# dvalcarce/filmyou-core

Hardware: AMD Instinct MI355X
Metric: top-N recs/sec (RM2), ml25m shape (higher is better)
Workload: dtype f32 (scores and logs fp32 / v_log_f32, folded in fp64; co-rating sums 64-bit fixed point in LDS (fp64 fallback); G stored as 24-bit e7m17 floats scaled per cluster above 4096 items; ratings fp16 in the row kernel when exactly representable)

## Files before the change

### filmyou-core_amd/csrc/fy_cooc.hpp

```cpp
#pragma once
#include <hip/hip_fp16.h>

#include <type_traits>

#include "fy_common.hpp"

namespace fy {

struct CoocArgs {
    const int32_t* __restrict__ rank_pair;
    const int32_t* __restrict__ pair_start;
    const int32_t* __restrict__ seg_ptr;
    const int2* __restrict__ seg;
    const float* __restrict__ seg_w;
    const int32_t* __restrict__ csr_idx;
    const float* __restrict__ csr_w;
    int32_t pbase;
    int32_t slot_base;
    int32_t Ic;
    int32_t CH;
    int32_t nch;
    int32_t row0;
    int32_t nrows;
    int32_t q0;
    int32_t nq;
    const int32_t* __restrict__ local_start;
    int32_t row_stride;
    const uint32_t* __restrict__ csr_pk;
    const int2* __restrict__ item_seg;
    uint32_t pk_bytes;
    const int32_t* __restrict__ item_id;
    int32_t half;
    double fx_scale;
    int32_t tail_row0, tail_chunks;
    int32_t item_grab;
    int32_t acc_quarter;
    int32_t acc32;
    int32_t half_rows, head_chunks;
};
__device__ __forceinline__ bool cooc_row_is_cut(const CoocArgs& A, int row) { return A.half && (A.half_rows == 0 || row < A.half_rows); }
__device__ __forceinline__ int cooc_acc_index(int c, int quarter) { return quarter ? (c & 3) * quarter + (c >> 2) : c; }

#ifndef FY_COOC_NB
#define FY_COOC_NB 8
#endif
extern __shared__ __attribute__((aligned(16))) double fy_cooc_acc[];

struct SegBatch {
    int2 d;
    float w;
};
static_assert(FY_COOC_NB == 8, "the segment groups of cooc_seg_slot are 8 segments long");
__device__ __forceinline__ int cooc_seg_slot(int s_begin, int batch, int wave, int nwaves, int lane) {
    return s_begin + ((((batch << 3) + (lane >> 3)) * nwaves + wave) << 3) + (lane & 7);
}
__device__ __forceinline__ SegBatch cooc_first_batch(const CoocArgs& A, int s_begin, int s_end) {
    const int lane = threadIdx.x & 63;
    const int wave = __builtin_amdgcn_readfirstlane(threadIdx.x >> 6);
    SegBatch B{make_int2(0, 0), 0.0f};
    const int s = cooc_seg_slot(s_begin, 0, wave, blockDim.x >> 6, lane);
    if (s < s_end) { B.d = A.seg[s]; B.w = A.seg_w[s]; }
    return B;
}

template <bool PK, class ACC>
__device__ __forceinline__ void cooc_accumulate_segments(const CoocArgs& A, ACC* __restrict__ acc, int s_begin, int s_end, int c0, SegBatch first,
                                                         int rmask = -1 ) {
    const int lane = threadIdx.x & 63;
    const int wave = __builtin_amdgcn_readfirstlane(threadIdx.x >> 6);
    const int nwaves = blockDim.x >> 6;
    const int32_t* __restrict__ csr_idx = A.csr_idx;
    const float* __restrict__ csr_w = A.csr_w;
    const uint32_t* __restrict__ csr_pk = A.csr_pk;
    constexpr int NB = FY_COOC_NB;
    struct Group {
        int L[NB];
        float W[NB];
        int idx[NB];
        float x[NB];
    };
    auto issue = [&](Group& G, const int2& d, float w, int g) __attribute__((always_inline)) {
#pragma unroll
        for (int q = 0; q < NB; q++) {
            const int F = __builtin_amdgcn_readlane(d.x, g + q);
            G.L[q] = __builtin_amdgcn_readlane(d.y, g + q);
            G.W[q] = __uint_as_float(__builtin_amdgcn_readlane(__float_as_uint(w), g + q));
            const int at = F + (lane < G.L[q] ? lane : 0);
            G.x[q] = 0.0f;
            if constexpr (PK) G.idx[q] = (int)csr_pk[at];
            else {
                G.idx[q] = csr_idx[at] - c0;
                G.x[q] = csr_w[at];
            }
        }
    };
    auto commit = [&](Group& G) __attribute__((always_inline)) {
        if constexpr (PK) {
#pragma unroll
            for (int q = 0; q < NB; q++) {
                const uint32_t pk = (uint32_t)G.idx[q];
                G.x[q] = __half2float(__ushort_as_half((unsigned short)(pk >> 16)));
                G.idx[q] = (int)(pk & 0xFFFFu);
            }
        }
#pragma unroll
        for (int q = 0; q < NB; q++)
            if (lane < G.L[q] && G.idx[q] > rmask) atomicAdd(&acc[cooc_acc_index(G.idx[q], A.acc_quarter)], (ACC)G.W[q] * (ACC)G.x[q]);
    };
    int batch = 0;
    if (cooc_seg_slot(s_begin, 0, wave, nwaves, 0) >= s_end) return;
    int2 d = first.d;
    float w = first.w;
    while (true) {
        const int nloc = __popcll(__ballot(cooc_seg_slot(s_begin, batch, wave, nwaves, lane) < s_end));
        const int s_next = cooc_seg_slot(s_begin, batch + 1, wave, nwaves, lane);
        int2 dn = make_int2(0, 0);
        float wn = 0.0f;
        if (s_next < s_end) { dn = A.seg[s_next]; wn = A.seg_w[s_next]; }
        Group GA, GB;
        issue(GA, d, w, 0);
#pragma unroll 1
        for (int g = 0; g < 64; g += 2 * NB) {
            issue(GB, d, w, g + NB);
            commit(GA);
            if (g + 2 * NB < 64) issue(GA, d, w, g + 2 * NB);
            commit(GB);
            if (g + 2 * NB >= nloc) break;
        }
        d = dn;
        w = wn;
        batch++;
        if (cooc_seg_slot(s_begin, batch, wave, nwaves, 0) >= s_end) break;
    }
}

struct PkGroup {
    int L[FY_COOC_NB];
    float W[FY_COOC_NB];
    uint32_t pk[FY_COOC_NB];
};
__device__ __forceinline__ void cooc_pk_issue(const __amdgpu_buffer_rsrc_t rsrc, int lane4, PkGroup& G, const int2& d, float w, int g) {
#pragma unroll
    for (int q = 0; q < FY_COOC_NB; q++) {
        const int F = __builtin_amdgcn_readlane(d.x, g + q);
        G.L[q] = __builtin_amdgcn_readlane(d.y, g + q);
        G.W[q] = __uint_as_float(__builtin_amdgcn_readlane(__float_as_uint(w), g + q));
        G.pk[q] = (uint32_t)__builtin_amdgcn_raw_buffer_load_b32(rsrc, lane4, F * 4, 0);
    }
}
__device__ __forceinline__ __amdgpu_buffer_rsrc_t cooc_pk_rsrc(const CoocArgs& A) {
    return __builtin_amdgcn_make_buffer_rsrc(const_cast<uint32_t*>(A.csr_pk), 0, (int)A.pk_bytes, 0x00020000);
}
template <class ACC>
__device__ __forceinline__ void cooc_accumulate_pk(const CoocArgs& A, ACC* __restrict__ acc, int s_begin, int s_end, SegBatch first,
                                                   int rmask = -1 ) {
    const int lane = threadIdx.x & 63;
    const int wave = __builtin_amdgcn_readfirstlane(threadIdx.x >> 6);
    const int nwaves = blockDim.x >> 6;
    const __amdgpu_buffer_rsrc_t rsrc = cooc_pk_rsrc(A);
    const int lane4 = lane * 4;
    constexpr int NB = FY_COOC_NB;
    using Group = PkGroup;
    auto issue = [&](Group& G, const int2& d, float w, int g) __attribute__((always_inline)) { cooc_pk_issue(rsrc, lane4, G, d, w, g); };
    const double fx = A.fx_scale;
    const uint32_t ix_mask = A.acc_quarter ? 3u : 0u, ix_shift = A.acc_quarter ? 2u : 0u, ix_quarter = (uint32_t)A.acc_quarter;
    auto commit = [&](Group& G) __attribute__((always_inline)) {
#pragma unroll
        for (int q = 0; q < NB; q++) {
            const float x = __half2float(__ushort_as_half((unsigned short)(G.pk[q] >> 16)));
            if constexpr (std::is_same<ACC, uint32_t>::value) {
                const uint32_t v = (uint32_t)(G.W[q] * x * (float)fx);
                if (lane < G.L[q] && (int)(G.pk[q] & 0xFFFFu) > rmask) atomicAdd(&acc[cooc_acc_index((int)(G.pk[q] & 0xFFFFu), A.acc_quarter)], v);
            } else if constexpr (std::is_same<ACC, unsigned long long>::value) {
                const double d = fma((double)(G.W[q] * x), fx, 4503599627370496.0);
                unsigned long long v = (unsigned long long)__double_as_longlong(d) & 0xFFFFFFFFFFFFFull;
                const uint32_t c = G.pk[q] & 0xFFFFu;
                uint32_t at = __umul24(c & ix_mask, ix_quarter) + (c >> ix_shift);
                asm volatile("" : "+v"(at), "+v"(v));
                if (lane < G.L[q] && (int)c > rmask) atomicAdd(&acc[at], v);
            } else {
                const ACC v = (ACC)(G.W[q] * x);
                if (lane < G.L[q] && (int)(G.pk[q] & 0xFFFFu) > rmask) atomicAdd(&acc[cooc_acc_index((int)(G.pk[q] & 0xFFFFu), A.acc_quarter)], v);
            }
        }
    };
    int batch = 0;
    if (cooc_seg_slot(s_begin, 0, wave, nwaves, 0) >= s_end) return;
    int2 d = first.d;
    float w = first.w;
    while (true) {
        const int nloc = __popcll(__ballot(cooc_seg_slot(s_begin, batch, wave, nwaves, lane) < s_end));
        const int s_next = cooc_seg_slot(s_begin, batch + 1, wave, nwaves, lane);
        int2 dn = make_int2(0, 0);
        float wn = 0.0f;
        if (s_next < s_end) { dn = A.seg[s_next]; wn = A.seg_w[s_next]; }
        Group GA, GB;
        issue(GA, d, w, 0);
#pragma unroll 1
        for (int g = 0; g < 64; g += 2 * NB) {
            issue(GB, d, w, g + NB);
            commit(GA);
            if (g + 2 * NB < 64) issue(GA, d, w, g + 2 * NB);
            commit(GB);
            if (g + 2 * NB >= nloc) break;
        }
        d = dn;
        w = wn;
        batch++;
        if (cooc_seg_slot(s_begin, batch, wave, nwaves, 0) >= s_end) break;
    }
}

template <bool PK = false>
__device__ __forceinline__ void cooc_accumulate_row(const CoocArgs& A, int row, int ch, int lrow = 0) {
    int s_begin, s_end;
    if (A.item_seg) {
        const int2 se = A.item_seg[(int64_t)lrow * A.nch + ch];
        s_begin = se.x;
        s_end = se.y;
    } else {
        const int pair = A.rank_pair[A.pbase + row];
        int e0 = A.pair_start[pair], e1 = A.pair_start[pair + 1];
        if (A.local_start) { e0 = A.local_start[lrow]; e1 = A.local_start[lrow + 1]; }
        const int32_t* __restrict__ sp = A.seg_ptr + (int64_t)ch * (A.nq + 1) - A.q0;
        s_begin = sp[e0];
        s_end = sp[e1];
    }
    if constexpr (PK) cooc_accumulate_pk<double>(A, fy_cooc_acc, s_begin, s_end, cooc_first_batch(A, s_begin, s_end));
    else cooc_accumulate_segments<false, double>(A, fy_cooc_acc, s_begin, s_end, ch * A.CH, cooc_first_batch(A, s_begin, s_end));
}

__attribute__((unused)) static __global__ void k_item_segments(CoocArgs A, int2* __restrict__ out) {
    const int n = A.nrows * A.nch;
    const int stride = A.row_stride ? A.row_stride : 1;
    for (int t = blockIdx.x * blockDim.x + threadIdx.x; t < n; t += gridDim.x * blockDim.x) {
        const int lrow = t / A.nch, ch = t % A.nch;
        const int pair = A.rank_pair[A.pbase + A.row0 + lrow * stride];
        int e0 = A.pair_start[pair], e1 = A.pair_start[pair + 1];
        if (A.local_start) { e0 = A.local_start[lrow]; e1 = A.local_start[lrow + 1]; }
        const int32_t* __restrict__ sp = A.seg_ptr + (int64_t)ch * (A.nq + 1) - A.q0;
        out[t] = make_int2(sp[e0], sp[e1]);
    }
}

__host__ __device__ inline int64_t cooc_half_item_index(int32_t row, int32_t ch, int32_t CH, int32_t nch) {
    const int64_t c = row / CH;
    return (int64_t)CH * (c * nch - c * (c - 1) / 2) + (int64_t)(row - c * CH) * (nch - c) + (ch - c);
}
inline int64_t cooc_item_count(int32_t nrows, int32_t CH, int32_t nch, bool half) {
    if (!half) return (int64_t)nrows * nch;
    return nrows > 0 ? cooc_half_item_index(nrows - 1, nch - 1, CH, nch) + 1 : 0;
}
__device__ __forceinline__ void item_list_body(const CoocArgs& A, int2* __restrict__ seg_out, int32_t* __restrict__ id_out) {
    const int n = A.nrows * A.nch;
    const int stride = A.row_stride ? A.row_stride : 1;
    for (int t = blockIdx.x * blockDim.x + threadIdx.x; t < n; t += gridDim.x * blockDim.x) {
        const int lrow = t / A.nch, ch = t % A.nch;
        const int row = A.row0 + lrow * stride;
        int64_t at = t;
        if (A.half && A.half_rows > 0) {
            if (row < A.half_rows) {
                if (ch < row / A.CH || ch >= A.head_chunks) continue;
                at = cooc_half_item_index(row, ch, A.CH, A.head_chunks);
            } else {
                if (ch >= A.tail_chunks) continue;
                at = cooc_half_item_index(A.half_rows - 1, A.head_chunks - 1, A.CH, A.head_chunks) + 1 + (int64_t)(row - A.half_rows) * A.tail_chunks + ch;
            }
        } else if (A.half) {
            if (ch < row / A.CH) continue;
            at = cooc_half_item_index(row, ch, A.CH, A.nch);
        } else if (A.tail_chunks > 0 && lrow >= A.tail_row0) {
            if (ch >= A.tail_chunks) continue;
            at = (int64_t)A.tail_row0 * A.nch + (int64_t)(lrow - A.tail_row0) * A.tail_chunks + ch;
        }
        const int pair = A.rank_pair[A.pbase + row];
        int e0 = A.pair_start[pair], e1 = A.pair_start[pair + 1];
        if (A.local_start) { e0 = A.local_start[lrow]; e1 = A.local_start[lrow + 1]; }
        const int32_t* __restrict__ sp = A.seg_ptr + (int64_t)ch * (A.nq + 1) - A.q0;
        seg_out[at] = make_int2(sp[e0], sp[e1]);
        id_out[at] = (lrow << 8) | ch;
    }
}
__attribute__((unused)) static __global__ void k_item_list(CoocArgs A, int2* __restrict__ seg_out, int32_t* __restrict__ id_out) {
    item_list_body(A, seg_out, id_out);
}

struct SegTable {
    int64_t n_seg = 0;
    DevBuf<int32_t> cnt, scratch;
    DevBuf<int32_t> ptr;
    DevBuf<int2> seg;
    DevBuf<float> w;
    const int32_t* v_ptr = nullptr;
    const int2* v_seg = nullptr;
    const float* v_w = nullptr;
    const int32_t* ptr_() const { return v_ptr ? v_ptr : ptr.get(); }
    const int2* seg_() const { return v_seg ? v_seg : seg.get(); }
    const float* w_() const { return v_w ? v_w : w.get(); }
};
void build_segments(Context* ctx, const int32_t* csc_slot, const float* csc_w, const int32_t* chunk_off, int32_t slot_base,
                    int32_t q0, int32_t nq, int32_t nch, SegTable& out, hipStream_t st = nullptr,
                    const int32_t* half_row_of_entry = nullptr, const int32_t* csr_idx = nullptr, int32_t CH = 0,
                    const int32_t* only_rows_of_entry = nullptr, int32_t only_rows_from = 0, int64_t max_segments = 0,
                    const int32_t* samples = nullptr);
void build_csr_samples(Context* ctx, int64_t nnz, const int32_t* csr_idx, DevBuf<int32_t>& samp, hipStream_t st = nullptr);

void build_chunk_offsets(Context* ctx, const int32_t* rowptr, const int32_t* csr_idx, int32_t slot_base, int32_t n_slots,
                         int32_t CH, int32_t nch, int32_t* chunk_off, hipStream_t st = nullptr);

__host__ __device__ inline int cooc_lds_columns(int CH) { return (CH % 256 == 0) ? CH : ((CH + 255) / 256) * 256 + 256; }

inline void pick_chunks(int32_t Ic, int32_t max_ch, int32_t& CH, int32_t& nch) {
    if (Ic <= max_ch) {
        CH = (int32_t)round_up(Ic > 0 ? Ic : 1, 64);
        nch = 1;
    } else {
        const int32_t cap = max_ch >= 256 ? (max_ch / 256) * 256 : max_ch;
        const int32_t gran = max_ch >= 256 ? 256 : 64;
        nch = (int32_t)ceil_div(Ic, cap);
        CH = (int32_t)std::min<int64_t>(cap, round_up(ceil_div(Ic, nch), gran));
        nch = (int32_t)ceil_div(Ic, CH);
    }
}

}
```

### filmyou-core_amd/csrc/fy_rm2.hip

```cpp
#include <algorithm>
#include <cmath>
#include <cstdlib>
#include <type_traits>

#include "fy_cooc.hpp"
#include "fy_prep.hpp"
#include <chrono>
#include "fy_rm2.hpp"

namespace fy {

static inline int grid_for(int64_t n, int block = 256, int cap = 256 * 16) {
    int64_t g = ceil_div(n, block);
    return (int)std::max<int64_t>(1, std::min<int64_t>(g, cap));
}

constexpr int PAIR_HEAVY = 2048;
struct PairPass {
    const int32_t* __restrict__ rank_pair;
    const int32_t* __restrict__ pair_start;
    const int32_t* __restrict__ pair_di;
    const int32_t* __restrict__ csc_slot;
    const float* __restrict__ csc_r;
    const double2* __restrict__ ud_slot;
// ... 87 lines not shown
    t.ps += x.ps; t.b += x.b; t.ws += x.ws; t.w += x.w;
    t.wm = fmaxf(t.wm, x.wm); t.rm = fmaxf(t.rm, x.rm);
}
__global__ __launch_bounds__(256) void k_pair_chunks(PairPass A, PairHeavy H) {
    __shared__ PairAcc sh_a[4];
    const int lane = threadIdx.x & 63, wave = threadIdx.x >> 6;
    const int n = H.counters[1];
    for (int c = blockIdx.x; c < n; c += gridDim.x) {
        const int32_t k = H.chunk_col[c];
        const int32_t pr = A.rank_pair[H.col[k]];
        const int32_t q0 = A.pair_start[pr] + (c - H.base[k]) * PAIR_CHUNK, q1 = min(A.pair_start[pr + 1], q0 + PAIR_CHUNK);
        PairAcc a = fy_pair_zero();
#pragma unroll 4
        for (int32_t q = q0 + (int32_t)threadIdx.x; q < q1; q += 256) fy_pair_entry(A, q, a);
        fy_pair_reduce(a);
        if (lane == 0) sh_a[wave] = a;
        __syncthreads();
        if (threadIdx.x == 0) {
            PairAcc t = sh_a[0];
            for (int x = 1; x < 4; x++) fy_pair_add(t, sh_a[x]);
            H.acc[c] = t;
        }
        __syncthreads();
    }
}
__global__ void k_pair_finish(PairPass A, PairHeavy H) {
    const int n = H.counters[0];
    for (int k = blockIdx.x * blockDim.x + threadIdx.x; k < n; k += gridDim.x * blockDim.x) {
        const int32_t pos = H.col[k], pr = A.rank_pair[pos];
        const int32_t len = A.pair_start[pr + 1] - A.pair_start[pr], nchk = (len + PAIR_CHUNK - 1) / PAIR_CHUNK;
        PairAcc t = H.acc[H.base[k]];
        for (int32_t i = 1; i < nchk; i++) fy_pair_add(t, H.acc[H.base[k] + i]);
        fy_pair_store(A, pos, pr, len, t);
    }
}
__global__ void k_slot_user_arrays(int32_t nU, const int32_t* __restrict__ slot2du, const double* __restrict__ usum,
                                   const int32_t* __restrict__ udeg, double* __restrict__ usum_slot, int32_t* __restrict__ deg_slot,
                                   double2* __restrict__ ud_slot) {
    for (int32_t s = blockIdx.x * blockDim.x + threadIdx.x; s < nU; s += gridDim.x * blockDim.x) {
        const int32_t du = slot2du[s];
        usum_slot[s] = usum[du];
        deg_slot[s] = udeg[du];
        ud_slot[s] = make_double2(usum[du], (double)udeg[du]);
    }
}

__global__ void k_cluster_fx_bounds(const int32_t* __restrict__ pcstart, const float* __restrict__ fx_rank, float* __restrict__ out) {
    const int c = blockIdx.x;
    float m0 = 0.f, m1 = 0.f, m2 = 0.f;
    for (int32_t pos = pcstart[c] + blockIdx.y * blockDim.x + threadIdx.x; pos < pcstart[c + 1]; pos += gridDim.y * blockDim.x) {
        m0 = fmaxf(m0, fx_rank[3 * (int64_t)pos]);
        m1 = fmaxf(m1, fx_rank[3 * (int64_t)pos + 1]);
        m2 = fmaxf(m2, fx_rank[3 * (int64_t)pos + 2]);
    }
    for (int o = 32; o > 0; o >>= 1) {
        m0 = fmaxf(m0, __shfl_down(m0, o, 64));
        m1 = fmaxf(m1, __shfl_down(m1, o, 64));
        m2 = fmaxf(m2, __shfl_down(m2, o, 64));
    }
    if ((threadIdx.x & 63) == 0) {
        if (m0 > 0.f) atomicMax(reinterpret_cast<int*>(out + 3 * c), __float_as_int(m0));
        if (m1 > 0.f) atomicMax(reinterpret_cast<int*>(out + 3 * c + 1), __float_as_int(m1));
        if (m2 > 0.f) atomicMax(reinterpret_cast<int*>(out + 3 * c + 2), __float_as_int(m2));
    }
}

__global__ void k_partial_total(int32_t lo, int32_t hi, const int32_t* __restrict__ slot2du, const double* __restrict__ usum,
                                unsigned long long* __restrict__ counter) {
    unsigned long long local = 0;
    for (int32_t s = lo + blockIdx.x * blockDim.x + threadIdx.x; s < hi; s += gridDim.x * blockDim.x)
        local += (unsigned long long)((long long)usum[slot2du[s]] * 100LL);
    for (int o = 32; o > 0; o >>= 1) local += __shfl_down(local, o, 64);
    __shared__ unsigned long long sh[16];
    if ((threadIdx.x & 63) == 0) sh[threadIdx.x >> 6] = local;
    __syncthreads();
    if (threadIdx.x == 0) {
        for (int w = 1; w < (int)(blockDim.x >> 6); w++) local += sh[w];
        if (local) atomicAdd(counter, local);
    }
}
__global__ void k_store_total(const unsigned long long* __restrict__ counter, double* __restrict__ dst) {
    *dst = (double)*counter;
}

__global__ void k_sum_gathered(int64_t len, int32_t world, const double* __restrict__ gathered, double* __restrict__ out) {
    for (int64_t d = blockIdx.x * (int64_t)blockDim.x + threadIdx.x; d < len; d += (int64_t)gridDim.x * blockDim.x) {
        double s = 0.0;
        for (int r = 0; r < world; r++) s += gathered[(int64_t)r * len + d];
        out[d] = s;
    }
}

__global__ void k_stats_to_raw(int32_t nI, const int32_t* __restrict__ iid, const double* __restrict__ partial, int64_t n_raw_items, int32_t nU,
                               const int32_t* __restrict__ uid, const double* __restrict__ usum, double* __restrict__ raw) {
    const int32_t n = max(nI + 1, nU);
    for (int32_t t = blockIdx.x * blockDim.x + threadIdx.x; t < n; t += gridDim.x * blockDim.x) {
        if (t < nI) raw[iid[t]] = partial[t];
        if (t == nI) raw[n_raw_items] = partial[nI];
        if (t < nU) raw[n_raw_items + 1 + uid[t]] = usum[t];
    }
}
__global__ void k_stats_from_raw(int32_t nI, const int32_t* __restrict__ iid, const double* __restrict__ raw, int64_t n_raw_items,
                                 double* __restrict__ stats) {
    for (int32_t t = blockIdx.x * blockDim.x + threadIdx.x; t <= nI; t += gridDim.x * blockDim.x) stats[t] = t < nI ? raw[iid[t]] : raw[n_raw_items];
}
__global__ void k_rank_flags(int32_t world, int64_t len, const double* __restrict__ gathered, double* __restrict__ out) {
    if ((int)threadIdx.x < world) out[threadIdx.x] = gathered[(int64_t)threadIdx.x * len + len - 1];
}
__global__ void k_flag_positive(int64_t n, const double* __restrict__ v, uint32_t* __restrict__ flag) {
    for (int64_t t = blockIdx.x * (int64_t)blockDim.x + threadIdx.x; t < n; t += (int64_t)gridDim.x * blockDim.x) flag[t] = v[t] > 0.0 ? 1u : 0u;
}
__global__ void k_compact_positive(int64_t n, const double* __restrict__ v, const uint32_t* __restrict__ pos, const double* __restrict__ divide_by,
                                   int32_t* __restrict__ id, double* __restrict__ val) {
    const double d = divide_by ? *divide_by : 1.0;
    for (int64_t t = blockIdx.x * (int64_t)blockDim.x + threadIdx.x; t < n; t += (int64_t)gridDim.x * blockDim.x)
        if (v[t] > 0.0) {
            id[pos[t] - 1] = (int32_t)t;
            val[pos[t] - 1] = divide_by ? v[t] / d : v[t];
        }
}

__global__ void k_item_coll(int32_t nI, const double* __restrict__ stats, double* __restrict__ icoll, double* __restrict__ total_out) {
    const double total = stats[nI] / 100.0;
    for (int32_t d = blockIdx.x * blockDim.x + threadIdx.x; d < nI; d += gridDim.x * blockDim.x) icoll[d] = stats[d] / total;
    if (blockIdx.x == 0 && threadIdx.x == 0) *total_out = total;
}

__global__ void k_pair_p(int32_t nP, const int32_t* __restrict__ rank_pair, const int32_t* __restrict__ pair_di,
                         const double* __restrict__ icoll, double lambda, const double* __restrict__ b_rank,
                         double* __restrict__ p_rank, float* __restrict__ a_rank, float* __restrict__ b_rank32, double2* __restrict__ pb_rank) {
    for (int32_t pos = blockIdx.x * blockDim.x + threadIdx.x; pos < nP; pos += gridDim.x * blockDim.x) {
        const double p = icoll[pair_di[rank_pair[pos]]];
        p_rank[pos] = p;
        pb_rank[pos] = make_double2(p, b_rank[pos]);
        a_rank[pos] = (float)(lambda * p);
        b_rank32[pos] = (float)b_rank[pos];
    }
}

__global__ void k_csc_x(int64_t nnz, const int32_t* __restrict__ csc_slot, const float* __restrict__ csc_r,
                        const double* __restrict__ usum_slot, float* __restrict__ csc_x, float* __restrict__ csc_x_over_s) {
    for (int64_t q = blockIdx.x * (int64_t)blockDim.x + threadIdx.x; q < nnz; q += (int64_t)gridDim.x * blockDim.x) {
        const double s = usum_slot[csc_slot[q]];
        const double x = (double)csc_r[q] / s;
        csc_x[q] = (float)x;
        if (csc_x_over_s) csc_x_over_s[q] = (float)(x / s);
    }
}

__global__ void k_csc_rank(int64_t nnz, const int32_t* __restrict__ csc_pair, const int32_t* __restrict__ pair_rank, int32_t* __restrict__ out) {
    for (int64_t q = blockIdx.x * (int64_t)blockDim.x + threadIdx.x; q < nnz; q += (int64_t)gridDim.x * blockDim.x) out[q] = pair_rank[csc_pair[q]];
}

__device__ __forceinline__ void pack_csr_body(int32_t f0, int32_t f1, int32_t CH, const int32_t* __restrict__ csr_idx, const float* __restrict__ csr_r,
                                              uint32_t* __restrict__ pk) {
    for (int64_t f = f0 + blockIdx.x * (int64_t)blockDim.x + threadIdx.x; f < f1; f += (int64_t)gridDim.x * blockDim.x)
        pk[f] = (uint32_t)(csr_idx[f] % CH) | ((uint32_t)__half_as_ushort(__float2half(csr_r[f])) << 16);
}
__global__ void k_pack_csr(int32_t f0, int32_t f1, int32_t CH, const int32_t* __restrict__ csr_idx, const float* __restrict__ csr_r,
                           uint32_t* __restrict__ pk) {
    pack_csr_body(f0, f1, CH, csr_idx, csr_r, pk);
}

__device__ __forceinline__ void tail_blocks_body(int32_t slot_base, int32_t n_slots, int32_t p_eff, const int32_t* __restrict__ rowptr,
                                                const int32_t* __restrict__ csr_idx, const float* __restrict__ csr_r, uint32_t* __restrict__ y_pk,
                                                int32_t* __restrict__ co2) {
    __shared__ int sh_count;
    const int lane = threadIdx.x & 63, wave = threadIdx.x >> 6;
    for (int32_t k = blockIdx.x; k < n_slots; k += gridDim.x) {
        const int32_t base = rowptr[slot_base + k], end = rowptr[slot_base + k + 1];
        int32_t lo = base, hi = end;
        while (lo < hi) { const int32_t mid = (lo + hi) >> 1; if (csr_idx[mid] < p_eff) lo = mid + 1; else hi = mid; }
        const int32_t first = lo;
        if (threadIdx.x == 0) sh_count = 0;
        __syncthreads();
        for (int32_t f0 = first + wave * 64; f0 < end; f0 += 4 * 64) {
            const int32_t f = f0 + lane;
            const int blk = f < end ? (csr_idx[f] - p_eff) >> 6 : -1;
            int prev = __shfl_up(blk, 1, 64);
            if (lane == 0) prev = f0 > first ? (csr_idx[f0 - 1] - p_eff) >> 6 : -1;
            const bool start = blk >= 0 && blk != prev;
            const unsigned long long bal = __ballot(start);
            int at = 0;
            if (lane == 0 && bal) at = atomicAdd(&sh_count, (int)__popcll(bal));
            at = __shfl(at, 0, 64);
            if (start) {
                float m = csr_r[f];
                for (int32_t g = f + 1; g < end && ((csr_idx[g] - p_eff) >> 6) == blk; g++) m = fmaxf(m, csr_r[g]);
                y_pk[base + at + __popcll(bal & ((1ull << lane) - 1ull))] = (uint32_t)blk | ((uint32_t)__half_as_ushort(__float2half(m)) << 16);
            }
        }
        __syncthreads();
        if (threadIdx.x == 0) { co2[2 * k] = base; co2[2 * k + 1] = base + sh_count; }
        __syncthreads();
    }
}
__global__ __launch_bounds__(256) void k_tail_blocks(int32_t slot_base, int32_t n_slots, int32_t p_eff, const int32_t* __restrict__ rowptr,
                                                     const int32_t* __restrict__ csr_idx, const float* __restrict__ csr_r, uint32_t* __restrict__ y_pk,
                                                     int32_t* __restrict__ co2) {
    tail_blocks_body(slot_base, n_slots, p_eff, rowptr, csr_idx, csr_r, y_pk, co2);
}

__global__ void k_csr_values(int32_t nU, const int32_t* __restrict__ rowptr, const int32_t* __restrict__ csr_idx,
                             const float* __restrict__ csr_r, const int32_t* __restrict__ slot2du,
                             const int32_t* __restrict__ ucluster, const double* __restrict__ usum,
                             const int32_t* __restrict__ csize, const int32_t* __restrict__ pcstart,
                             const double2* __restrict__ pb_rank, double lambda,
                             const float* __restrict__ gscale ,
                             float* __restrict__ csr_x, float* __restrict__ csr_e, float* __restrict__ csr_q) {
    const int lane = threadIdx.x & 63;
    const int wpb = blockDim.x >> 6;
    for (int32_t s = blockIdx.x * wpb + (threadIdx.x >> 6); s < nU; s += gridDim.x * wpb) {
        const int32_t du = slot2du[s];
        const int32_t c = ucluster[du];
        const double sum = usum[du];
        const double Uc1 = (double)(csize[c] - 1);
        const double gs = (double)gscale[c];
        const int32_t pb = pcstart[c];
        for (int32_t f = rowptr[s] + lane; f < rowptr[s + 1]; f += 64) {
            const int32_t j = csr_idx[f];
            const double x = (double)csr_r[f] / sum;
            const double2 pbj = pb_rank[pb + j];
            double e = (1.0 - lambda) * (pbj.y - x) + lambda * Uc1 * pbj.x;
            if (!(e > 0.0)) e = 0.0;
            csr_x[f] = (float)x;
            csr_e[f] = (float)(e * gs);
            csr_q[f] = (float)(lambda * (1.0 - lambda) * pbj.x * gs);
        }
    }
}

__global__ void k_user_meta(int32_t lo, int32_t hi, const int32_t* __restrict__ slot2du, const int32_t* __restrict__ uid,
                            const int32_t* __restrict__ ucluster, const int32_t* __restrict__ udeg,
                            const int32_t* __restrict__ csize, const int32_t* __restrict__ pcstart, int32_t number_of_items,
                            int32_t top_n, int32_t filter_users, const int32_t* __restrict__ cshift ,
                            double* __restrict__ pvpi, int32_t* __restrict__ n_out,
                            unsigned long long* __restrict__ counters ) {
    unsigned long long terms = 0, scored = 0;
    for (int32_t s = lo + blockIdx.x * blockDim.x + threadIdx.x; s < hi; s += gridDim.x * blockDim.x) {
        const int32_t du = slot2du[s];
        const int32_t c = ucluster[du];
        const int32_t n = udeg[du];
        const int32_t Ic = pcstart[c + 1] - pcstart[c];
        const int32_t unrated = Ic - n;
        pvpi[s - lo] = (double)(n - 1) * log((double)number_of_items) - (double)n * log((double)csize[c]) +
                       (double)n * (double)cshift[c] * 0.69314718055994530942;
        const bool skip = unrated <= 0 || uid[du] < filter_users;
        int32_t k = skip ? 0 : min(top_n, unrated);
        if (k < 0) k = 0;
        n_out[s - lo] = k;
        if (!skip) { terms += (unsigned long long)n * (unsigned long long)unrated; scored++; }
    }
    for (int o = 32; o > 0; o >>= 1) {
        terms += __shfl_down(terms, o, 64);
        scored += __shfl_down(scored, o, 64);
    }
    if ((threadIdx.x & 63) == 0) {
        if (terms) atomicAdd(&counters[0], terms);
        if (scored) atomicAdd(&counters[1], scored);
    }
}

__device__ __forceinline__ void chunk_offsets_body(const int32_t* __restrict__ rowptr, const int32_t* __restrict__ csr_idx, int32_t slot_base,
                                                   int32_t n_slots, int32_t CH, int32_t nch, int32_t* __restrict__ chunk_off) {
    const int64_t total = (int64_t)n_slots * (nch + 1);
    for (int64_t t = blockIdx.x * (int64_t)blockDim.x + threadIdx.x; t < total; t += (int64_t)gridDim.x * blockDim.x) {
        const int32_t v = (int32_t)(t / (nch + 1)), ch = (int32_t)(t % (nch + 1));
        const int32_t a = rowptr[slot_base + v], b = rowptr[slot_base + v + 1];
        int32_t lo = a, hi = b;
        const int32_t key = ch * CH;
        while (lo < hi) {
            const int32_t mid = (lo + hi) >> 1;
            if (csr_idx[mid] < key) lo = mid + 1; else hi = mid;
        }
        chunk_off[t] = (ch == nch) ? b : lo;
    }
}
__global__ void k_chunk_offsets(const int32_t* __restrict__ rowptr, const int32_t* __restrict__ csr_idx, int32_t slot_base,
                                int32_t n_slots, int32_t CH, int32_t nch, int32_t* __restrict__ chunk_off) {
    chunk_offsets_body(rowptr, csr_idx, slot_base, n_slots, CH, nch, chunk_off);
}

void build_chunk_offsets(Context* ctx, const int32_t* rowptr, const int32_t* csr_idx, int32_t slot_base, int32_t n_slots,
                         int32_t CH, int32_t nch, int32_t* chunk_off, hipStream_t st) {
    const int64_t total = (int64_t)n_slots * (nch + 1);
    if (total == 0) return;
    k_chunk_offsets<<<grid_for(total), 256, 0, st ? st : ctx->stream>>>(rowptr, csr_idx, slot_base, n_slots, CH, nch, chunk_off);
    FY_KERNEL_CHECK();
}

#ifndef FY_SAMPLE_SHIFT
#define FY_SAMPLE_SHIFT 6
#endif
struct Half {
    const int32_t* __restrict__ row_of_entry;
    const int32_t* __restrict__ csr_idx;
    int32_t CH;
    int32_t* __restrict__ start;
    const int32_t* __restrict__ samp;
    const int32_t* __restrict__ only_rows;
    int32_t only_from;
    int32_t sym_rows, lim_from, lim_chunks;
};
__device__ __forceinline__ void seg_counts_body(const int32_t* __restrict__ csc_slot, const int32_t* __restrict__ chunk_off, int32_t slot_base,
                                                int32_t q0, int32_t nq, int32_t nch, int32_t* __restrict__ cnt, const Half& H) {
    const bool row4 = nch == 3 && (reinterpret_cast<uintptr_t>(chunk_off) & 15) == 0;
    const bool row2 = nch == 1 && (reinterpret_cast<uintptr_t>(chunk_off) & 7) == 0;
    for (int64_t q = blockIdx.x * (int64_t)blockDim.x + threadIdx.x; q <= nq; q += (int64_t)gridDim.x * blockDim.x) {
        const bool live = q < nq && !(H.only_rows && H.only_rows[q0 + q] < H.only_from);
        const int32_t* co = live ? chunk_off + (int64_t)(csc_slot[q0 + q] - slot_base) * (nch + 1) : nullptr;
        int4 c4 = make_int4(0, 0, 0, 0);
        if (live && row4) c4 = *reinterpret_cast<const int4*>(co);
        if (live && row2) { const int2 v = *reinterpret_cast<const int2*>(co); c4.x = v.x; c4.y = v.y; }
        auto CO = [&](int k) -> int32_t { return (row4 || row2) ? (k == 0 ? c4.x : k == 1 ? c4.y : k == 2 ? c4.z : c4.w) : co[k]; };
        int32_t prev = live ? CO(0) : 0;
        int32_t own = -1, behind = 0, climit = nch;
        const int32_t r_e = (live && H.row_of_entry) ? H.row_of_entry[q0 + q] : 0;
        if (live && H.row_of_entry && H.lim_chunks > 0 && r_e >= H.lim_from) climit = H.lim_chunks;
        if (live && H.row_of_entry && (H.sym_rows == 0 || r_e < H.sym_rows)) {
            const int32_t r = r_e;
            own = r / H.CH;
            constexpr int SS = FY_SAMPLE_SHIFT;
            const int32_t co_own = CO(own), co_next = CO(own + 1);
            int32_t klo = (co_own + (1 << SS) - 1) >> SS, khi = (co_next + (1 << SS) - 1) >> SS;
            while (klo < khi) {
                const int32_t mid = (klo + khi) >> 1;
                if (H.samp[mid] <= r) klo = mid + 1; else khi = mid;
            }
            const int32_t lo = max(co_own, (klo - 1) << SS);
            behind = lo;
            H.start[q] = lo;
        }
        for (int32_t ch = 0; ch < nch; ch++) {
            int32_t n = 0;
            if (live) {
                const int32_t next = CO(ch + 1);
                const int32_t first = ch == own ? behind : prev;
                n = (ch < own || ch >= climit) ? 0 : (next - first + 63) >> 6;
                prev = next;
            }
            cnt[(int64_t)ch * (nq + 1) + q] = n;
        }
    }
}
__global__ void k_seg_counts(const int32_t* __restrict__ csc_slot, const int32_t* __restrict__ chunk_off, int32_t slot_base,
                             int32_t q0, int32_t nq, int32_t nch, int32_t* __restrict__ cnt, Half H) {
    seg_counts_body(csc_slot, chunk_off, slot_base, q0, nq, nch, cnt, H);
}
struct SegDesc {
    int32_t slot_base, q0, nq, nch, CH, half, only_from, co_stride;
    int64_t co_off, cnt_off;
    int32_t use_only_rows, sym_rows;
    int32_t lim_from, lim_chunks;
};
__global__ void k_seg_counts_multi(const SegDesc* __restrict__ D, const int32_t* __restrict__ csc_slot, const int32_t* __restrict__ co_all,
                                   int32_t* __restrict__ cnt_all, const int32_t* __restrict__ row_of_entry, const int32_t* __restrict__ csr_idx,
                                   int32_t* __restrict__ start_all, const int32_t* __restrict__ samples) {
    const SegDesc d = D[blockIdx.y];
    const Half H{(d.half || d.lim_chunks > 0) ? row_of_entry : nullptr, csr_idx, d.CH, start_all + d.q0, samples, d.use_only_rows ? row_of_entry : nullptr, d.only_from,
                 d.half ? d.sym_rows : -1, d.lim_from, d.lim_chunks};
    seg_counts_body(csc_slot, co_all + d.co_off, d.slot_base, d.q0, d.nq, d.nch, cnt_all + d.cnt_off, H);
}

__device__ __forceinline__ void seg_fill_body(const int32_t* __restrict__ csc_slot, const float* __restrict__ csc_w, const int32_t* __restrict__ chunk_off,
                                              int32_t slot_base, int32_t q0, int32_t nq, int32_t nch, const int32_t* __restrict__ ptr,
                                              int2* __restrict__ seg, float* __restrict__ seg_w, const Half& H) {
    constexpr int CB = 4;
    const bool row4 = nch == 3 && (reinterpret_cast<uintptr_t>(chunk_off) & 15) == 0;
    const bool row2 = nch == 1 && (reinterpret_cast<uintptr_t>(chunk_off) & 7) == 0;
    const int lane = threadIdx.x & 63, wpb = blockDim.x >> 6;
    const int64_t n_groups = ((int64_t)nq + 63) >> 6;
    const int32_t n_cb = (nch + CB - 1) / CB;
    const int64_t total_work = n_groups * n_cb;
    for (int64_t gw = blockIdx.x * (int64_t)wpb + (threadIdx.x >> 6); gw < total_work; gw += (int64_t)gridDim.x * wpb) {
        const int32_t ch0 = (int32_t)(gw / n_groups) * CB;
        const int64_t g = gw - (int64_t)(ch0 / CB) * n_groups;
        const int64_t q = g * 64 + lane;
        const int64_t q_end = min((int64_t)nq, g * 64 + 64);
        const bool live = q < nq;
        int32_t cov[CB + 1], startv[CB], endv[CB];
        int32_t r = 0, own = -1, own_start = 0;
        bool dead = false, limited = false;
        float w = 0.0f;
#pragma unroll
        for (int c = 0; c < CB; c++) {
            startv[c] = 0;
            endv[c] = ch0 + c < nch ? ptr[(int64_t)(ch0 + c) * (nq + 1) + q_end] : 0;
            if (live && ch0 + c < nch) startv[c] = ptr[(int64_t)(ch0 + c) * (nq + 1) + q];
        }
#pragma unroll
        for (int c = 0; c <= CB; c++) cov[c] = 0;
        if (live) {
            const int32_t* co = chunk_off + (int64_t)(csc_slot[q0 + q] - slot_base) * (nch + 1) + ch0;
            if (row4) {
                const int4 v = *reinterpret_cast<const int4*>(co);
                cov[0] = v.x; cov[1] = v.y; cov[2] = v.z; cov[3] = v.w;
            } else if (row2) {
                const int2 v = *reinterpret_cast<const int2*>(co);
                cov[0] = v.x; cov[1] = v.y;
            } else {
#pragma unroll
                for (int c = 0; c <= CB; c++)
                    if (ch0 + c <= nch) cov[c] = co[c];
            }
            if (H.row_of_entry) {
                r = H.row_of_entry[q0 + q];
                if (H.sym_rows == 0 || r < H.sym_rows) {
                    own = r / H.CH;
                    if (own >= ch0 && own < ch0 + CB) own_start = H.start[q];
                }
                limited = H.lim_chunks > 0 && r >= H.lim_from;
            }
            if (H.only_rows && H.only_rows[q0 + q] < H.only_from) dead = true;
            w = csc_w[q0 + q];
        }
#pragma unroll
        for (int c = 0; c < CB; c++) {
            const int32_t ch = ch0 + c;
            if (ch >= nch) break;
            int32_t f0 = cov[c], len = cov[c + 1] - cov[c], start = startv[c];
            if (live) {
                if (own >= 0) {
                    if (ch < own) len = 0;
                    else if (ch == own) { f0 = own_start; len = cov[c + 1] - f0; }
                }
                if (limited && ch >= H.lim_chunks) len = 0;
                if (dead) len = 0;
            } else len = 0;
            const int32_t base = __shfl(start, 0, 64);
            const int32_t total = endv[c] - base;
            if (!live) start = base + total;
            const int32_t rel = start - base;
            for (int32_t kk = 0; kk < total; kk += 64) {
                const int32_t k = kk + lane;
                int lo = 0, hi = 63;
#pragma unroll
                for (int it = 0; it < 6; it++) {
                    const int mid = (lo + hi + 1) >> 1;
                    const int32_t rm = __shfl(rel, mid, 64);
                    if (rm <= k) lo = mid; else hi = mid - 1;
                }
                const int32_t off = k - __shfl(rel, lo, 64);
                const int32_t of0 = __shfl(f0, lo, 64), olen = __shfl(len, lo, 64);
                const float ow = __shfl(w, lo, 64);
                if (k < total) {
                    seg[base + k] = make_int2(of0 + 64 * off, min(64, olen - 64 * off));
                    seg_w[base + k] = ow;
                }
            }
        }
    }
}

__global__ void k_seg_fill(const int32_t* __restrict__ csc_slot, const float* __restrict__ csc_w, const int32_t* __restrict__ chunk_off,
                           int32_t slot_base, int32_t q0, int32_t nq, int32_t nch, const int32_t* __restrict__ ptr,
                           int2* __restrict__ seg, float* __restrict__ seg_w, Half H) {
    seg_fill_body(csc_slot, csc_w, chunk_off, slot_base, q0, nq, nch, ptr, seg, seg_w, H);
}
__global__ void k_seg_fill_multi(const SegDesc* __restrict__ D, const int32_t* __restrict__ csc_slot, const float* __restrict__ csc_w,
                                 const int32_t* __restrict__ co_all, const int32_t* __restrict__ ptr_all, int2* __restrict__ seg, float* __restrict__ seg_w,
                                 const int32_t* __restrict__ row_of_entry, const int32_t* __restrict__ csr_idx, int32_t* __restrict__ start_all) {
    const SegDesc d = D[blockIdx.y];
    const Half H{(d.half || d.lim_chunks > 0) ? row_of_entry : nullptr, csr_idx, d.CH, start_all + d.q0, nullptr, d.use_only_rows ? row_of_entry : nullptr, d.only_from,
                 d.half ? d.sym_rows : -1, d.lim_from, d.lim_chunks};
    seg_fill_body(csc_slot, csc_w, co_all + d.co_off, d.slot_base, d.q0, d.nq, d.nch, ptr_all + d.cnt_off, seg, seg_w, H);
}
struct CoDesc {
    int32_t slot_base, n_slots, CH, nch, f0, f1, p_eff, has_tail;
    int64_t co_off, co_tail_off;
};
__global__ void k_chunk_offsets_multi(const CoDesc* __restrict__ D, const int32_t* __restrict__ rowptr, const int32_t* __restrict__ csr_idx,
                                      int32_t* __restrict__ co_all) {
    const CoDesc d = D[blockIdx.y];
    chunk_offsets_body(rowptr, csr_idx, d.slot_base, d.n_slots, d.CH, d.nch, co_all + d.co_off);
}
__global__ void k_pack_csr_multi(const CoDesc* __restrict__ D, const int32_t* __restrict__ csr_idx, const float* __restrict__ csr_r, uint32_t* __restrict__ pk) {
    const CoDesc d = D[blockIdx.y];
    pack_csr_body(d.f0, d.f1, d.CH, csr_idx, csr_r, pk);
}
__global__ __launch_bounds__(256) void k_tail_blocks_multi(const CoDesc* __restrict__ D, const int32_t* __restrict__ rowptr, const int32_t* __restrict__ csr_idx,
                                                           const float* __restrict__ csr_r, uint32_t* __restrict__ y_pk, int32_t* __restrict__ co_tail_all) {
    const CoDesc d = D[blockIdx.y];
    if (!d.has_tail) return;
    tail_blocks_body(d.slot_base, d.n_slots, d.p_eff, rowptr, csr_idx, csr_r, y_pk, co_tail_all + d.co_tail_off);
}
__global__ void k_csr_samples(int64_t n_samples, const int32_t* __restrict__ csr_idx, int32_t* __restrict__ samp) {
    for (int64_t k = blockIdx.x * (int64_t)blockDim.x + threadIdx.x; k < n_samples; k += (int64_t)gridDim.x * blockDim.x) samp[k] = csr_idx[k << FY_SAMPLE_SHIFT];
}
void build_csr_samples(Context* ctx, int64_t nnz, const int32_t* csr_idx, DevBuf<int32_t>& samp, hipStream_t st) {
    const int64_t n = (nnz + (1 << FY_SAMPLE_SHIFT) - 1) >> FY_SAMPLE_SHIFT;
    samp.alloc(ctx, (size_t)n + 1);
    if (n) k_csr_samples<<<grid_for(n), 256, 0, st ? st : ctx->stream>>>(n, csr_idx, samp.get());
    FY_KERNEL_CHECK();
}
void build_segments(Context* ctx, const int32_t* csc_slot, const float* csc_w, const int32_t* chunk_off, int32_t slot_base,
                    int32_t q0, int32_t nq, int32_t nch, SegTable& out, hipStream_t st, const int32_t* half_row_of_entry,
                    const int32_t* csr_idx, int32_t CH, const int32_t* only_rows_of_entry, int32_t only_rows_from, int64_t max_segments,
                    const int32_t* samples) {
    if (half_row_of_entry && !samples) FY_FAIL(FY_ERR_STATE, "internal: the symmetric segment table needs the CSR samples");
    if (!st) st = ctx->stream;
    const size_t np = (size_t)nch * ((size_t)nq + 1);
    out.ptr.alloc(ctx, np);
    out.cnt.alloc(ctx, np);
    out.scratch.alloc(ctx, half_row_of_entry ? (size_t)nq + 1 : 1);
    const Half H{half_row_of_entry, csr_idx, CH, out.scratch.get(), samples, only_rows_of_entry, only_rows_from};
    k_seg_counts<<<grid_for((int64_t)nq + 1), 256, 0, st>>>(csc_slot, chunk_off, slot_base, q0, nq, nch, out.cnt.get(), H);
    FY_KERNEL_CHECK();
    exclusive_scan_i32(ctx, out.cnt.get(), out.ptr.get(), np, st);
    int64_t total = max_segments;
    if (max_segments <= 0) {
        int32_t t32 = 0;
        FY_HIP(hipMemcpyAsync(&t32, out.ptr.get() + (np - 1), sizeof(int32_t), hipMemcpyDeviceToHost, st));
        FY_HIP(hipStreamSynchronize(st));
        total = t32;
    }
    out.n_seg = total;
    out.seg.alloc(ctx, (size_t)total);
    out.w.alloc(ctx, (size_t)total);
    if ((int64_t)nch * nq > 0) {
        k_seg_fill<<<grid_for((((int64_t)nq + 63) >> 6) * nch * 64, 256, 256 * 64), 256, 0, st>>>(csc_slot, csc_w, chunk_off, slot_base, q0, nq, nch, out.ptr.get(),
                                                                 out.seg.get(), out.w.get(), H);
        FY_KERNEL_CHECK();
    }
    if (max_segments <= 0) FY_HIP(hipStreamSynchronize(st));
}

constexpr int FY_P24_SHIFT = 6;
struct MEpilogue {
    float* __restrict__ M;
    int64_t ldm;
    float w2;
    double fx_inv;
    int pack24;
    float* __restrict__ Bmax;
    int64_t ldb;
    int local_rows;
    int32_t panel_cols;
    float* __restrict__ Bmax64;
    int64_t ldb64;
    uint32_t* __restrict__ Brep;
    int64_t pitch;
    int ceil24;
    double* __restrict__ head32;
    int64_t ld_head;
    int32_t head_rows;
    double* __restrict__ tail32;
    int32_t tail_from;
};

template <class ACC, bool COPY>
__device__ __forceinline__ void cooc_rm2_epilogue_pack(const CoocArgs& A, const MEpilogue& E, ACC* __restrict__ acc, int row, int mrow, int c0, int c1, int cb,
                                                       int first_bmax_block) {
        const int64_t row_cols = E.pitch ? E.pitch : (E.panel_cols ? E.panel_cols : E.ldm);
        const uint32_t radd = E.ceil24 ? (1u << FY_P24_SHIFT) - 1u : 1u << (FY_P24_SHIFT - 1);
        uint32_t* __restrict__ out3 = reinterpret_cast<uint32_t*>(reinterpret_cast<char*>(E.M) + (int64_t)mrow * row_cols * 3);
        for (int c4 = (cb >> 2) + threadIdx.x; 4 * c4 < c1; c4 += blockDim.x) {
            uint32_t v[4];
            const int qz = A.acc_quarter;
            ACC* ap = acc + (qz ? c4 - (c0 >> 2) : 4 * c4 - c0);
            const int qs = qz ? qz : 1;
            double f4[COPY ? 4 : 1];
#pragma unroll
            for (int q = 0; q < 4; q++) {
                float f;
                if constexpr (std::is_integral<ACC>::value) { const double d = (double)ap[q * qs] * E.fx_inv; f = (float)d; if constexpr (COPY) f4[q] = d; }
                else { f = E.w2 * (float)ap[q * qs]; if constexpr (COPY) f4[q] = (double)E.w2 * (double)ap[q * qs]; }
                ap[q * qs] = (ACC)0;
                v[q] = (__float_as_uint(f) + radd) >> FY_P24_SHIFT;
            }
            if constexpr (COPY) {
            if (E.head32 && mrow < E.head_rows && 4 * c4 < E.ld_head) {
                double2* hp = reinterpret_cast<double2*>(E.head32 + (int64_t)mrow * E.ld_head + 4 * c4);
                hp[0] = make_double2(f4[0], f4[1]);
                hp[1] = make_double2(f4[2], f4[3]);
            }
            if (E.tail32 && row >= E.tail_from && 4 * c4 < E.head_rows) {
                double2* tp = reinterpret_cast<double2*>(E.tail32 + (int64_t)(row - E.tail_from) * E.head_rows + 4 * c4);
                tp[0] = make_double2(f4[0], f4[1]);
                tp[1] = make_double2(f4[2], f4[3]);
            }
            }
            if (!E.panel_cols || 4 * c4 < E.panel_cols) {
                out3[3 * c4 + 0] = v[0] | (v[1] << 24);
                out3[3 * c4 + 1] = (v[1] >> 8) | (v[2] << 16);
                out3[3 * c4 + 2] = (v[2] >> 16) | (v[3] << 8);
            }
            if (E.Bmax64) {
                const uint32_t cq = (uint32_t)((4 * c4) & 63);
                const uint32_t k0 = (v[0] << 6) | cq, k1 = (v[1] << 6) | (cq + 1), k2 = (v[2] << 6) | (cq + 2), k3 = (v[3] << 6) | (cq + 3);
                const uint32_t a1 = max(k0, k1), a2 = min(k0, k1), b1 = max(k2, k3), b2 = min(k2, k3);
                uint32_t t1 = max(a1, b1), t2 = max(min(a1, b1), max(a2, b2));
#define FY_ROR16(x, n) ((uint32_t)__builtin_amdgcn_update_dpp(0, (int)(x), 0x120 + (n), 0xF, 0xF, false))
#define FY_TOP2_STEP(n)                                         \
    {                                                           \
        const uint32_t p1 = FY_ROR16(t1, n), p2 = FY_ROR16(t2, n); \
        t2 = max(min(t1, p1), max(t2, p2));                     \
        t1 = max(t1, p1);                                       \
    }
                FY_TOP2_STEP(8) FY_TOP2_STEP(4) FY_TOP2_STEP(2) FY_TOP2_STEP(1)
#undef FY_TOP2_STEP
#undef FY_ROR16
                const uint32_t m = t1 >> 6;
                if ((threadIdx.x & 15) == 0 && m) {
                    uint8_t* bp = reinterpret_cast<uint8_t*>(E.Bmax64) + ((int64_t)mrow * E.ldb64 + (c4 >> 4)) * 3;
                    bp[0] = (uint8_t)m;
                    bp[1] = (uint8_t)(m >> 8);
                    bp[2] = (uint8_t)(m >> 16);
                    if (E.Brep) E.Brep[(int64_t)mrow * E.ldb64 + (c4 >> 4)] = ((t2 >> 6) << 8) | (t1 & 63u);
                }
            }
            if (E.Bmax) {
                uint32_t m = max(max(v[0], v[1]), max(v[2], v[3]));
#pragma unroll
                for (int o = 1; o < 64; o <<= 1) m = max(m, (uint32_t)__shfl_xor((int)m, o, 64));
                if ((threadIdx.x & 63) == 0 && m && (c4 >> 6) >= first_bmax_block) {
                    uint8_t* bp = reinterpret_cast<uint8_t*>(E.Bmax) + ((int64_t)mrow * E.ldb + (c4 >> 6)) * 3;
                    bp[0] = (uint8_t)m;
                    bp[1] = (uint8_t)(m >> 8);
                    bp[2] = (uint8_t)(m >> 16);
                }
            }
        }
}

template <class ACC>
__device__ __forceinline__ void cooc_rm2_epilogue(const CoocArgs& A, const MEpilogue& E, ACC* __restrict__ acc, int id) {
    const int lrow = id >> 8;
    const int row = A.row0 + lrow * (A.row_stride ? A.row_stride : 1);
    const int mrow = E.local_rows ? lrow : row;
    const int ch = id & 255;
    const int c0 = ch * A.CH;
    const int c1 = (ch == A.nch - 1) ? (int)E.ldm : min(c0 + A.CH, (int)E.ldm);
    const int cb = (cooc_row_is_cut(A, row) && c0 <= row) ? (row & ~255) : c0;
    const int first_bmax_block = A.half ? (row >> 8) + 1 : 0;
    if (E.pack24) {
        const bool copy = E.head32 && (mrow < E.head_rows || (E.tail32 && row >= E.tail_from && c0 < E.head_rows));
        if (copy) cooc_rm2_epilogue_pack<ACC, true>(A, E, acc, row, mrow, c0, c1, cb, first_bmax_block);
        else cooc_rm2_epilogue_pack<ACC, false>(A, E, acc, row, mrow, c0, c1, cb, first_bmax_block);
    } else {
        float* __restrict__ out = E.M + (int64_t)mrow * E.ldm;
        for (int col = cb + threadIdx.x; col < c1; col += blockDim.x) {
            const int at = cooc_acc_index(col - c0, A.acc_quarter);
            if constexpr (std::is_integral<ACC>::value) out[col] = (float)((double)acc[at] * E.fx_inv);
            else out[col] = E.w2 * (float)acc[at];
            acc[at] = (ACC)0;
        }
    }
}

template <bool PK, class ACC>
__device__ __forceinline__ void cooc_rm2_body(const CoocArgs& A, const MEpilogue& E, int n_items, int* __restrict__ next_item) {
    ACC* __restrict__ acc = reinterpret_cast<ACC*>(fy_cooc_acc);
    __shared__ int sh_item, sh_s0, sh_s1, sh_id;
    const int CHp = cooc_lds_columns(A.CH);
    for (int t = threadIdx.x; t < CHp; t += blockDim.x) acc[t] = (ACC)0;
    const int ITEM_GRAB = A.item_grab > 0 ? A.item_grab : 1;
    int next = 0, next2 = 0;
    int g_cur = 0, g_end = 0, g_next = 0;
    auto grab = [&]() __attribute__((always_inline)) {
        if (g_cur == g_end) {
            g_cur = g_next;
            g_end = g_cur + ITEM_GRAB;
            g_next = atomicAdd(next_item, ITEM_GRAB);
        }
        return g_cur++;
    };
    if (threadIdx.x == 0) {
        g_cur = atomicAdd(next_item, ITEM_GRAB);
        g_end = g_cur + ITEM_GRAB;
        g_next = atomicAdd(next_item, ITEM_GRAB);
        const int first = grab();
        next = grab();
        const int2 se = first < n_items ? A.item_seg[first] : make_int2(0, 0);
        sh_item = first;
        sh_s0 = se.x;
        sh_s1 = se.y;
        sh_id = first < n_items ? A.item_id[first] : 0;
    }
    __syncthreads();
    int item = sh_item, s0 = sh_s0, s1 = sh_s1, id = sh_id;
    __syncthreads();
    SegBatch batch = cooc_first_batch(A, s0, s1);
    while (item < n_items) {
        int2 se_next = make_int2(0, 0);
        int id_next = 0;
        if (threadIdx.x == 0) {
            next2 = grab();
            if (next < n_items) { se_next = A.item_seg[next]; id_next = A.item_id[next]; }
        }
        const int c0 = (id & 255) * A.CH;
        const int row_of_item = A.row0 + (id >> 8) * (A.row_stride ? A.row_stride : 1);
        const int rmask = (cooc_row_is_cut(A, row_of_item) && row_of_item >= c0 && row_of_item < c0 + A.CH) ? row_of_item - c0 : -1;
        if constexpr (PK) cooc_accumulate_pk<ACC>(A, acc, s0, s1, batch, rmask);
        else cooc_accumulate_segments<false, ACC>(A, acc, s0, s1, c0, batch, rmask);
        if (threadIdx.x == 0) { sh_item = next; sh_s0 = se_next.x; sh_s1 = se_next.y; sh_id = id_next; }
        __syncthreads();
        const int nitem = sh_item;
        s0 = sh_s0;
        s1 = sh_s1;
        const int nid = sh_id;
        batch = cooc_first_batch(A, s0, s1);
        cooc_rm2_epilogue<ACC>(A, E, acc, id);
        item = nitem;
        id = nid;
        if (threadIdx.x == 0) next = next2;
        __syncthreads();
    }
}
template <bool PK, class ACC, int ROLE = 0>
__global__ void k_cooc_rm2(CoocArgs A, MEpilogue E, int n_items, int* __restrict__ next_item) {
    cooc_rm2_body<PK, ACC>(A, E, n_items, next_item);
}
struct CoocLaunch {
    CoocArgs A;
    MEpilogue E;
    int32_t n_items, pad;
};
template <bool PK, class ACC, int ROLE = 0>
__global__ void k_cooc_rm2_multi(const CoocLaunch* __restrict__ D, int* __restrict__ counters) {
    const CoocLaunch& d = D[blockIdx.y];
    const CoocArgs A = d.A;
    const MEpilogue E = d.E;
    cooc_rm2_body<PK, ACC>(A, E, d.n_items, counters + blockIdx.y);
}
__global__ void k_item_list_multi(const CoocLaunch* __restrict__ D) {
    const CoocArgs A = D[blockIdx.y].A;
    item_list_body(A, const_cast<int2*>(A.item_seg), const_cast<int32_t*>(A.item_id));
}

__device__ __forceinline__ void fy_unpack24_raw(uint32_t d0, uint32_t d1, uint32_t d2, uint32_t* v) {
    v[0] = d0 & 0xFFFFFFu;
    v[1] = (d0 >> 24) | ((d1 & 0xFFFFu) << 8);
    v[2] = (d1 >> 16) | ((d2 & 0xFFu) << 16);
    v[3] = d2 >> 8;
}
__device__ __forceinline__ uint32_t fy_load24(const uint32_t* __restrict__ row3, int e) {
    const int g = e >> 2;
    uint32_t v[4];
    fy_unpack24_raw(row3[3 * g], row3[3 * g + 1], row3[3 * g + 2], v);
    return v[e & 3];
}
constexpr int MIRROR_PITCH = 772;

extern __shared__ __attribute__((aligned(16))) unsigned char fy_mirror_lds[];
__device__ __forceinline__ void mirror_tiles_body(float* __restrict__ M_, int64_t ldm, int32_t Ic, float* __restrict__ Bmax_, int64_t ldb,
                                                  const int32_t* __restrict__ need = nullptr, int32_t write_below = 0x7FFFFFFF) {
    __shared__ uint32_t rowmax[128];
    const int tj = blockIdx.x, B = blockIdx.y;
    if (tj < 2 * (B + 1)) return;
    const int dst_row0 = 128 * tj;
    if (dst_row0 >= Ic) return;
    const bool write = B < write_below || (need && need[B] != 0);
    if (!write && !Bmax_) return;
    const int lane = threadIdx.x & 63, wave = threadIdx.x >> 6, nwaves = blockDim.x >> 6;
    const int64_t pitch = ldm * 3;
    unsigned char* __restrict__ Mb = reinterpret_cast<unsigned char*>(M_);
    if (threadIdx.x < 128) rowmax[threadIdx.x] = 0;
    __syncthreads();
    const int m = lane & 31, h = lane >> 5;
    uint32_t mx[4] = {0, 0, 0, 0};
    for (int r = 2 * wave + h; r < 256; r += 2 * nwaves) {
        const int src_row = 256 * B + r;
        uint32_t v[4] = {0, 0, 0, 0};
        if (src_row < Ic) {
            const uint32_t* __restrict__ p = reinterpret_cast<const uint32_t*>(Mb + (int64_t)src_row * pitch + (int64_t)dst_row0 * 3) + 3 * m;
            fy_unpack24_raw(p[0], p[1], p[2], v);
        }
#pragma unroll
        for (int q = 0; q < 4; q++) {
            if (write) {
                unsigned char* d = fy_mirror_lds + (4 * m + q) * MIRROR_PITCH + 3 * r;
                d[0] = (unsigned char)v[q];
                d[1] = (unsigned char)(v[q] >> 8);
                d[2] = (unsigned char)(v[q] >> 16);
            }
            mx[q] = max(mx[q], v[q]);
        }
    }
#pragma unroll
    for (int q = 0; q < 4; q++)
        if (mx[q]) atomicMax(&rowmax[4 * m + q], mx[q]);
    __syncthreads();
    for (int c = wave; write && c < 128; c += nwaves) {
        const int dst_row = dst_row0 + c;
        if (dst_row >= Ic) break;
        const uint32_t* __restrict__ sp = reinterpret_cast<const uint32_t*>(fy_mirror_lds + c * MIRROR_PITCH) + 3 * lane;
        uint32_t* __restrict__ dp = reinterpret_cast<uint32_t*>(Mb + (int64_t)dst_row * pitch + (int64_t)256 * B * 3) + 3 * lane;
        dp[0] = sp[0];
        dp[1] = sp[1];
        dp[2] = sp[2];
    }
    if (Bmax_ && threadIdx.x < 128 && dst_row0 + (int)threadIdx.x < Ic) {
        const uint32_t pv = rowmax[threadIdx.x];
        uint8_t* bp = reinterpret_cast<uint8_t*>(Bmax_) + ((int64_t)(dst_row0 + threadIdx.x) * ldb + B) * 3;
        bp[0] = (uint8_t)pv;
        bp[1] = (uint8_t)(pv >> 8);
        bp[2] = (uint8_t)(pv >> 16);
    }
}

__global__ __launch_bounds__(1024) void k_mirror_tiles(float* __restrict__ M_, int64_t ldm, int32_t Ic, float* __restrict__ Bmax_, int64_t ldb,
                                                       const int32_t* __restrict__ need, int32_t write_below) {
    mirror_tiles_body(M_, ldm, Ic, Bmax_, ldb, need, write_below);
}
__global__ __launch_bounds__(1024) void k_colmax_upper(const float* __restrict__ M_, int64_t ldm, int32_t Ic, float* __restrict__ Bmax_, int64_t ldb, int32_t first_block) {
    __shared__ uint32_t colmax[256];
    const int tj = blockIdx.x, B = first_block + blockIdx.y;
    if (tj <= B) return;
    const int col0 = 256 * tj;
    if (col0 >= Ic) return;
    const int lane = threadIdx.x & 63, wave = threadIdx.x >> 6;
    const int64_t pitch = ldm * 3;
    const unsigned char* __restrict__ Mb = reinterpret_cast<const unsigned char*>(M_);
    if (threadIdx.x < 256) colmax[threadIdx.x] = 0;
    __syncthreads();
    uint32_t mx[4] = {0, 0, 0, 0};
    const int r_end = min(256, Ic - 256 * B);
    uint32_t d[4][3];
#pragma unroll
    for (int step = 0; step < 4; step++) {
#pragma unroll
        for (int x = 0; x < 4; x++) {
            const int r = wave * 16 + step * 4 + x;
            const uint32_t* __restrict__ p = reinterpret_cast<const uint32_t*>(Mb + (int64_t)(256 * B + min(r, r_end - 1)) * pitch + (int64_t)col0 * 3) + 3 * lane;
            d[x][0] = p[0]; d[x][1] = p[1]; d[x][2] = p[2];
        }
#pragma unroll
        for (int x = 0; x < 4; x++) {
            uint32_t v[4];
            fy_unpack24_raw(d[x][0], d[x][1], d[x][2], v);
#pragma unroll
            for (int q = 0; q < 4; q++) mx[q] = max(mx[q], v[q]);
        }
    }
#pragma unroll
    for (int q = 0; q < 4; q++)
        if (mx[q]) atomicMax(&colmax[4 * lane + q], mx[q]);
    __syncthreads();
    if (threadIdx.x < 256 && col0 + (int)threadIdx.x < Ic) {
        const uint32_t pv = colmax[threadIdx.x];
        uint8_t* bp = reinterpret_cast<uint8_t*>(Bmax_) + ((int64_t)(col0 + threadIdx.x) * ldb + B) * 3;
        bp[0] = (uint8_t)pv;
        bp[1] = (uint8_t)(pv >> 8);
        bp[2] = (uint8_t)(pv >> 16);
    }
}
__global__ void k_flag_surviving_blocks(int32_t n_users, const int32_t* __restrict__ n_quads, const uint16_t* __restrict__ surv, int64_t ldb, int32_t* __restrict__ need) {
// ... 42 lines not shown
struct PanelDesc {
    float* Gp;
    float* Bmax64;
    uint32_t* Brep;
    int64_t panel_cols, ldb64;
    int32_t Ic, p_eff, nsub, pad;
};
__global__ __launch_bounds__(1024) void k_mirror_tiles_multi(const PanelDesc* __restrict__ D) {
    const PanelDesc d = D[blockIdx.z];
    if ((int)blockIdx.x >= (int)(d.panel_cols / 128) || (int)blockIdx.y >= (int)(d.panel_cols / 256) - 1) return;
    mirror_tiles_body(d.Gp, d.panel_cols, d.p_eff, nullptr, 0);
}
__global__ __launch_bounds__(256) void k_mirror_diag_multi(const PanelDesc* __restrict__ D) {
    const PanelDesc d = D[blockIdx.y];
    if ((int)blockIdx.x >= (int)(d.panel_cols / 256)) return;
    mirror_diag_body(d.Gp, d.panel_cols, d.p_eff, nullptr, 0);
}
__global__ __launch_bounds__(256) void k_panel_colmax(const PanelDesc* __restrict__ D) {
    const PanelDesc dsc = D[blockIdx.z];
    const float* __restrict__ Gp_ = dsc.Gp;
    float* __restrict__ Bmax64_ = dsc.Bmax64;
    uint32_t* __restrict__ Brep = dsc.Brep;
    const int64_t panel_cols = dsc.panel_cols, ldb64 = dsc.ldb64;
    const int32_t Ic = dsc.Ic, p_eff = dsc.p_eff, nsub = dsc.nsub;
    if ((int)blockIdx.x * 256 >= p_eff || (int)blockIdx.y * 16 >= nsub) return;
    __shared__ uint32_t sh_m[16][257], sh_r[16][257];
    const int lane = threadIdx.x & 63, wave = threadIdx.x >> 6;
    const int col0 = blockIdx.x * 256, sbg = blockIdx.y * 16;
    const int c = col0 + 4 * lane;
    const unsigned char* __restrict__ base = reinterpret_cast<const unsigned char*>(Gp_) + (int64_t)c * 3;
    const int64_t pitch = panel_cols * 3;
    for (int s = 0; s < 4; s++) {
        const int sb = sbg + 4 * wave + s;
        uint32_t t1[4] = {0, 0, 0, 0}, t2[4] = {0, 0, 0, 0};
        if (sb < nsub) {
            const int j0 = 64 * sb, nr = min(64, Ic - j0);
            for (int r = 0; r < nr; r += 8) {
                uint32_t d[8][3];
#pragma unroll
                for (int x = 0; x < 8; x++) {
                    const uint32_t* __restrict__ p = reinterpret_cast<const uint32_t*>(base + (int64_t)(j0 + min(r + x, nr - 1)) * pitch);
                    d[x][0] = p[0]; d[x][1] = p[1]; d[x][2] = p[2];
                }
#pragma unroll
                for (int x = 0; x < 8; x++) {
                    if (r + x < nr) {
                        uint32_t v[4];
                        fy_unpack24_raw(d[x][0], d[x][1], d[x][2], v);
#pragma unroll
                        for (int q = 0; q < 4; q++) {
                            const uint32_t key = (v[q] << 6) | (uint32_t)(r + x);
                            t2[q] = max(min(t1[q], key), t2[q]);
                            t1[q] = max(t1[q], key);
                        }
                    }
                }
            }
        }
#pragma unroll
        for (int q = 0; q < 4; q++) {
            sh_m[4 * wave + s][4 * lane + q] = t1[q] >> 6;
            sh_r[4 * wave + s][4 * lane + q] = (t1[q] >> 6) ? (((t2[q] >> 6) << 8) | (t1[q] & 63u)) : 0u;
        }
    }
    __syncthreads();
    const int i = col0 + threadIdx.x;
    if (i < p_eff) {
        uint32_t m[16];
#pragma unroll
        for (int k = 0; k < 16; k++) m[k] = sh_m[k][threadIdx.x];
        uint32_t* __restrict__ bp = reinterpret_cast<uint32_t*>(reinterpret_cast<unsigned char*>(Bmax64_) + ((int64_t)i * ldb64 + sbg) * 3);
#pragma unroll
        for (int g = 0; g < 4; g++) {
            const uint32_t* v = m + 4 * g;
            bp[3 * g + 0] = v[0] | (v[1] << 24);
            bp[3 * g + 1] = (v[1] >> 8) | (v[2] << 16);
            bp[3 * g + 2] = (v[2] >> 16) | (v[3] << 8);
        }
        uint32_t* __restrict__ rp = Brep + (int64_t)i * ldb64 + sbg;
#pragma unroll
        for (int k = 0; k < 16; k++) rp[k] = sh_r[k][threadIdx.x];
    }
}

static void launch_mirror(Context* ctx, float* M, int64_t ldm, int32_t Ic, float* Bmax, int64_t ldb, hipStream_t st, const int32_t* need = nullptr,
                          int32_t write_below = 0x7FFFFFFF, bool diag = true) {
    const int nblk = (int)(ldm / 256), ntile = (int)(ldm / 128);
    if (nblk > 1) {
        FY_HIP(hipFuncSetAttribute(reinterpret_cast<const void*>(k_mirror_tiles), hipFuncAttributeMaxDynamicSharedMemorySize, 128 * MIRROR_PITCH));
        const bool split = !need && Bmax && write_below < nblk - 1;
        const int ny = split ? write_below : nblk - 1;
        if (ny > 0) {
            k_mirror_tiles<<<dim3(ntile, ny), 1024, 128 * MIRROR_PITCH, st>>>(M, ldm, Ic, Bmax, ldb, need, write_below);
            FY_KERNEL_CHECK();
        }
        if (split) {
            k_colmax_upper<<<dim3(nblk, nblk - 1 - write_below), 1024, 0, st>>>(M, ldm, Ic, Bmax, ldb, write_below);
            FY_KERNEL_CHECK();
        }
    }
    if (diag) {
        k_mirror_diag<<<nblk, 256, 0, st>>>(M, ldm, Ic, Bmax, ldb);
        FY_KERNEL_CHECK();
    }
}

static void cooc_rm2_allow_lds() {
    const int bytes = 160 * 1024 - 256;
    FY_HIP(hipFuncSetAttribute(reinterpret_cast<const void*>(k_cooc_rm2<false, double>), hipFuncAttributeMaxDynamicSharedMemorySize, bytes));
    FY_HIP(hipFuncSetAttribute(reinterpret_cast<const void*>(k_cooc_rm2<true, double>), hipFuncAttributeMaxDynamicSharedMemorySize, bytes));
    FY_HIP(hipFuncSetAttribute(reinterpret_cast<const void*>(k_cooc_rm2<false, float>), hipFuncAttributeMaxDynamicSharedMemorySize, bytes));
    FY_HIP(hipFuncSetAttribute(reinterpret_cast<const void*>(k_cooc_rm2<true, float>), hipFuncAttributeMaxDynamicSharedMemorySize, bytes));
    FY_HIP(hipFuncSetAttribute(reinterpret_cast<const void*>(k_cooc_rm2<true, unsigned long long>), hipFuncAttributeMaxDynamicSharedMemorySize, bytes));
    FY_HIP(hipFuncSetAttribute(reinterpret_cast<const void*>(k_cooc_rm2<true, uint32_t>), hipFuncAttributeMaxDynamicSharedMemorySize, bytes));
    FY_HIP(hipFuncSetAttribute(reinterpret_cast<const void*>(k_cooc_rm2<true, unsigned long long, 1>), hipFuncAttributeMaxDynamicSharedMemorySize, bytes));
    FY_HIP(hipFuncSetAttribute(reinterpret_cast<const void*>(k_cooc_rm2_multi<true, unsigned long long, 0>), hipFuncAttributeMaxDynamicSharedMemorySize, bytes));
    FY_HIP(hipFuncSetAttribute(reinterpret_cast<const void*>(k_cooc_rm2_multi<true, unsigned long long, 1>), hipFuncAttributeMaxDynamicSharedMemorySize, bytes));
}
static void stray_allow_lds();

#include "fy_rm2_kernels.hpp"

static void stray_allow_lds() {
    FY_HIP(hipFuncSetAttribute(reinterpret_cast<const void*>(k_score_stray), hipFuncAttributeMaxDynamicSharedMemorySize, (STRAY_UCAP + 1) * (int)sizeof(int32_t)));
}

void launch_topn_rows(Context* ctx, hipStream_t st, const float* S, int64_t ldS, int32_t n_cols, int32_t n_rows,
                      const int32_t* n_out, const int32_t* out_off, const int32_t* rank_item_raw, const int32_t* slot2du,
                      const int32_t* uid, int32_t slot0, int32_t aux_value, int32_t* out_user, int32_t* out_item,
                      float* out_score, int32_t* out_aux, int32_t* overflow, int32_t* any_overflow, int32_t top_n_hint) {
    if (n_rows <= 0) return;
    if (!st) st = ctx->stream;
    TopNArgs TA{S, ldS, n_cols, n_out, out_off, rank_item_raw, slot2du, uid, slot0, slot0, aux_value, out_user, out_item, out_score, out_aux,
                0, 0, nullptr, nullptr, 0, nullptr, nullptr, nullptr};
    FY_HIP(hipMemsetAsync(any_overflow, 0, sizeof(int32_t), st));
    if (top_n_hint > TOPN_LONG) k_topn_long<<<n_rows, 256, (size_t)fy_topn_long_cap(top_n_hint) * 8, st>>>(TA, overflow, any_overflow, 0, fy_topn_long_cap(top_n_hint));
    else k_topn_fast<<<n_rows, 256, 0, st>>>(TA, overflow, any_overflow, 0);
    FY_KERNEL_CHECK();
    k_topn_select<<<n_rows, 256, 0, st>>>(TA, overflow, any_overflow);
    FY_KERNEL_CHECK();
}

}

using namespace fy;

struct TableCache {
    bool valid = false;
    int64_t total_segments = 0;
    std::vector<int32_t> sig;
    bool have_x = false;
    DevBuf<float> csc_x, csc_x_over_s;
    DevBuf<uint32_t> csr_pk, y_pk;
    DevBuf<int32_t> csc_rank, samples;
    std::vector<SegTable> segs, segs_tail;
    DevBuf<int32_t> g_co, g_co_tail, g_cnt, g_ptr, g_start;
    DevBuf<int2> g_seg;
    DevBuf<float> g_w;
};
struct RM2Static {
    int32_t K = 0, rank = 0, world = 1;
    int32_t max_item = -1;
    bool has_count = false;
    std::vector<int32_t> map_user, map_cluster, cluster_count;
    Prepared P;
    int32_t slot_lo = 0, slot_hi = 0;
    DevBuf<double> partial;
    bool sharded = false;
    int64_t n_raw_users = 0, n_raw_items = 0;
    std::vector<int32_t> owner;
    DevBuf<double> partial_raw;
    int deferred_code = 0;
    std::string deferred_msg;
    int64_t exchange_len() const { return sharded ? n_raw_items + 1 + n_raw_users + 1 : (int64_t)P.nI + 1; }
    DevBuf<double> b_rank, usum_slot;
    DevBuf<long long> walk_rank;
    DevBuf<int32_t> cnt_rank, deg_slot;
    DevBuf<float> fx_rank;
    std::vector<float> fx_bounds;
    double ms_build = 0;
    TableCache tables;
    bool matches(const fy_rm2_params* prm, int64_t n_map, const int32_t* mu, const int32_t* mc, const int32_t* cc) const {
        if (K != prm->number_of_clusters || rank != prm->rank || world != prm->world || (int64_t)map_user.size() != n_map || has_count != (cc != nullptr)) return false;
        if (n_map && (memcmp(map_user.data(), mu, (size_t)n_map * 4) || memcmp(map_cluster.data(), mc, (size_t)n_map * 4))) return false;
        if (cc && memcmp(cluster_count.data(), cc, (size_t)K * 4)) return false;
        return true;
    }
};

struct fy_rm2_job {
    Context* ctx = nullptr;
    fy_rm2_params prm{};
    std::shared_ptr<RM2Static> S;
    Prepared& P;
    int32_t &slot_lo, &slot_hi;
    DevBuf<double>& partial;
    DevBuf<double> stats;
    DevBuf<double> stats_raw;
    bool have_global = false;
    double ms_prepare = 0;
    bool from_cache = false;
    fy_collectives coll{};
    bool have_coll = false;
    DevBuf<double> gathered;
    DevBuf<double>&b_rank, &usum_slot;
    DevBuf<long long>& walk_rank;
    DevBuf<int32_t>&cnt_rank, &deg_slot;
    DevBuf<float>& fx_rank;
    std::vector<float>& fx_bounds;
    bool count_balanced = false;
    explicit fy_rm2_job(std::shared_ptr<RM2Static> s)
        : S(std::move(s)), P(S->P), slot_lo(S->slot_lo), slot_hi(S->slot_hi), partial(S->partial), b_rank(S->b_rank), usum_slot(S->usum_slot),
          walk_rank(S->walk_rank), cnt_rank(S->cnt_rank), deg_slot(S->deg_slot), fx_rank(S->fx_rank), fx_bounds(S->fx_bounds) {}
};

static void owner_range(const fy_rm2_job* J, int k, int32_t& lo, int32_t& hi) {
    if (J->S->sharded) { lo = 0; hi = k == J->prm.rank ? J->P.nU : 0; return; }
    if (!J->count_balanced) { rank_slot_range(J->P, k, J->prm.world, lo, hi); return; }
    const int64_t n = J->P.nU, W = J->prm.world;
    lo = (int32_t)(n * k / W);
    hi = (int32_t)(n * (k + 1) / W);
}

using ScoreTune = fy::Tuning;
static inline const ScoreTune& score_tune(const Context* ctx) { return ctx->tune; }

static int fx_exponent(const float* bounds3) {
    const double wsum = bounds3[0], wmax = bounds3[1], rmax = bounds3[2];
    if (!(wsum > 0.0) || !(wmax > 0.0) || !(rmax > 0.0) || !std::isfinite(wsum * rmax)) return -1;
    const int k1 = 51 - (std::ilogb(wmax * rmax) + 1), k2 = 62 - (std::ilogb(wsum * rmax) + 1);
    const int k = std::min(std::min(k1, k2), 1000);
    return k >= 24 ? k : -1;
}

static int cooc_item_grab(int64_t visits, int64_t n_items) { return n_items > 0 && visits / n_items < 12000 ? 8 : 1; }

static void launch_cooc_rm2(Context* ctx, const ScoreTune& tune, bool use_pk, const CoocArgs& CA_, const MEpilogue& ME, int n_items,
                            int32_t* counter, hipStream_t st) {
    if (n_items <= 0) return;
    CoocArgs CA = CA_;
    CA.acc_quarter = tune.cooc_planes ? cooc_lds_columns(CA.CH) / 4 : 0;
    const bool acc32 = CA.acc32 && use_pk && CA.fx_scale > 0.0 && !tune.cooc_f32;
    const size_t lds = (size_t)cooc_lds_columns(CA.CH) * ((tune.cooc_f32 || acc32) ? 4 : 8);
    const int by_lds = (int)std::max<size_t>(1, (160 * 1024 - 512) / (lds + 64));
    int block = tune.cooc_block;
    if (!block) block = by_lds >= 4 ? 256 : (by_lds >= 2 ? 512 : 1024);
    const int per_cu = std::max(1, std::min(by_lds, 2048 / block));
    const int grid = std::min(n_items, ctx->num_cus * per_cu);
    if (acc32) {
        k_cooc_rm2<true, uint32_t><<<grid, block, lds, st>>>(CA, ME, n_items, counter);
    } else if (use_pk && CA.fx_scale > 0.0 && !tune.cooc_f32) {
        if (ME.ceil24) k_cooc_rm2<true, unsigned long long, 1><<<grid, block, lds, st>>>(CA, ME, n_items, counter);
        else k_cooc_rm2<true, unsigned long long><<<grid, block, lds, st>>>(CA, ME, n_items, counter);
    } else if (!tune.cooc_f32) {
        if (use_pk) k_cooc_rm2<true, double><<<grid, block, lds, st>>>(CA, ME, n_items, counter);
        else k_cooc_rm2<false, double><<<grid, block, lds, st>>>(CA, ME, n_items, counter);
    } else {
        if (use_pk) k_cooc_rm2<true, float><<<grid, block, lds, st>>>(CA, ME, n_items, counter);
        else k_cooc_rm2<false, float><<<grid, block, lds, st>>>(CA, ME, n_items, counter);
    }
    FY_KERNEL_CHECK();
}

bool fy::gram_half_build(Context* ctx, const Prepared& P, const float* csc_w, const float* bounds3, float* G, int64_t ldm, double* ms_tables,
                         double* ms_walk) {
    const ScoreTune tune = score_tune(ctx);
    const int32_t Ic = P.nP;
    if (P.K != 1 || !P.ratings_fp16_exact || !P.ratings_positive || Ic <= 0) return false;
    int fxk = fx_exponent(bounds3);
    if (fxk < 0) return false;
    const int m = P.ratings_frac_bits;
    const bool acc32 = tune.isim_acc32 && m <= 4 && (double)bounds3[2] * bounds3[2] * std::ldexp(1.0, 2 * m) < 16777216.0 &&
                       (double)bounds3[0] * bounds3[2] * std::ldexp(1.0, 2 * m) < 4294967296.0;
    if (acc32) fxk = 2 * m;
    int32_t CH, nch;
    pick_chunks(Ic, acc32 && !tune.cooc_max_ch_forced ? 2 * tune.cooc_max_ch : tune.cooc_max_ch, CH, nch);
    if (nch >= 256) return false;
    hipStream_t st = ctx->stream;
    cooc_rm2_allow_lds();
    EventTimer t_tab(ctx), t_walk(ctx);
    const size_t s0 = t_tab.begin();
    DevBuf<uint32_t> csr_pk(ctx, (size_t)P.nnz);
    k_pack_csr<<<grid_for(P.nnz), 256, 0, st>>>(0, (int32_t)P.nnz, CH, P.csr_idx.get(), P.csr_r.get(), csr_pk.get());
    FY_KERNEL_CHECK();
    DevBuf<int32_t> co(ctx, (size_t)P.nU * (nch + 1)), csc_rank(ctx, (size_t)P.nnz);
    build_chunk_offsets(ctx, P.rowptr.get(), P.csr_idx.get(), 0, P.nU, CH, nch, co.get(), st);
    k_csc_rank<<<grid_for(P.nnz), 256, 0, st>>>(P.nnz, P.csc_pair.get(), P.pair_rank.get(), csc_rank.get());
    FY_KERNEL_CHECK();
    SegTable segs;
    DevBuf<int32_t> samples;
    build_csr_samples(ctx, P.nnz, P.csr_idx.get(), samples, st);
    build_segments(ctx, P.csc_slot.get(), csc_w, co.get(), 0, 0, (int32_t)P.nnz, nch, segs, st, csc_rank.get(), P.csr_idx.get(), CH, nullptr, 0, 0, samples.get());
    CoocArgs CA{P.rank_pair.get(), P.pair_start.get(), segs.ptr.get(), segs.seg.get(), segs.w.get(), P.csr_idx.get(), nullptr, 0, 0, Ic, CH, nch,
                0, Ic, 0, (int32_t)P.nnz, nullptr, 0, csr_pk.get(), nullptr, (uint32_t)std::min<int64_t>((int64_t)P.nnz * 4, 0xFFFFFFFFll)};
    CA.half = 1;
    CA.fx_scale = std::ldexp(1.0, fxk);
    CA.acc32 = acc32 ? 1 : 0;
    const int n_items = (int)cooc_item_count(Ic, CH, nch, true);
    DevBuf<int2> item_seg(ctx, (size_t)Ic * nch);
    DevBuf<int32_t> item_id(ctx, (size_t)Ic * nch), counter(ctx, 1);
    k_item_list<<<grid_for((int64_t)Ic * nch), 256, 0, st>>>(CA, item_seg.get(), item_id.get());
    FY_KERNEL_CHECK();
    CA.item_seg = item_seg.get();
    CA.item_id = item_id.get();
    counter.zero();
    CA.item_grab = cooc_item_grab(P.sum_deg2 / 2, n_items);
    MEpilogue ME{};
    ME.M = G;
    ME.ldm = ldm;
    ME.w2 = 1.0f;
    ME.fx_inv = std::ldexp(1.0, -fxk);
    t_tab.end(s0);
    const size_t s1 = t_walk.begin();
    launch_cooc_rm2(ctx, tune, true, CA, ME, n_items, counter.get(), st);
    t_walk.end(s1);
    sync(ctx);
    if (ms_tables) *ms_tables = t_tab.total_ms();
    if (ms_walk) *ms_walk = t_walk.total_ms();
    return true;
}

static void launch_cooc_rm2_multi(Context* ctx, const ScoreTune& tune, std::vector<CoocLaunch>& L, bool tail_role, DevBuf<CoocLaunch>& d_launch,
                                  DevBuf<int32_t>& d_counters, hipStream_t st, bool item_lists = false ) {
    if (L.empty()) return;
    int max_chp = 0, max_items = 0, max_list = 0;
    for (size_t k = 0; k < L.size(); k++)
        if (!L[k].A.item_seg || !L[k].A.item_id || !L[k].E.M || !L[k].A.seg || !L[k].A.seg_ptr || (L[k].E.panel_cols && !L[k].E.Bmax64))
            FY_FAIL(FY_ERR_STATE, "internal: launch %zu of %zu of a batched row kernel has a null operand (item_seg %p item_id %p M %p seg %p ptr %p Bmax64 %p)", k, L.size(),
                    (const void*)L[k].A.item_seg, (const void*)L[k].A.item_id, (const void*)L[k].E.M, (const void*)L[k].A.seg, (const void*)L[k].A.seg_ptr, (const void*)L[k].E.Bmax64);
    for (auto& x : L) {
        x.A.acc_quarter = tune.cooc_planes ? cooc_lds_columns(x.A.CH) / 4 : 0;
        max_chp = std::max(max_chp, cooc_lds_columns(x.A.CH));
        max_items = std::max(max_items, x.n_items);
        max_list = std::max(max_list, x.A.nrows * x.A.nch);
    }
    const size_t lds = (size_t)max_chp * 8;
    const int by_lds = (int)std::max<size_t>(1, (160 * 1024 - 512) / (lds + 64));
    int block = tune.cooc_block;
    if (!block) block = by_lds >= 4 ? 256 : (by_lds >= 2 ? 512 : 1024);
    const int per_cu = std::max(1, std::min(by_lds, 2048 / block));
    const int gx = std::max(1, std::min(max_items, ctx->num_cus * per_cu));
    d_launch.alloc(ctx, L.size());
    d_counters.alloc(ctx, L.size());
    FY_HIP(hipMemcpyAsync(d_launch.get(), L.data(), L.size() * sizeof(CoocLaunch), hipMemcpyHostToDevice, st));
    FY_HIP(hipMemsetAsync(d_counters.get(), 0, L.size() * sizeof(int32_t), st));
    const dim3 grid((unsigned)gx, (unsigned)L.size());
    if (item_lists) {
        k_item_list_multi<<<dim3((unsigned)std::max(1, std::min(grid_for(max_list), 4096)), (unsigned)L.size()), 256, 0, st>>>(d_launch.get());
        FY_KERNEL_CHECK();
    }
    if (tail_role) k_cooc_rm2_multi<true, unsigned long long, 1><<<grid, block, lds, st>>>(d_launch.get(), d_counters.get());
    else k_cooc_rm2_multi<true, unsigned long long, 0><<<grid, block, lds, st>>>(d_launch.get(), d_counters.get());
    FY_KERNEL_CHECK();
}

static int score_slices(const Context* ctx, const ScoreTune& tune, int64_t nb, int chunks) {
    const int64_t coarse = ceil_div(nb, 4 * (int64_t)tune.users_per_wave), finest = ceil_div(nb, 4);
    const int64_t fill = ceil_div(8 * (int64_t)ctx->num_cus, std::max(1, chunks));
    return (int)std::max<int64_t>(1, std::min<int64_t>(tune.max_slices, std::min(finest, std::max(coarse, fill))));
}

static void sup_block_map(int seed_blocks, int nblk, std::vector<int32_t>& first) {
    first.clear();
    const int R = std::max(0, nblk - seed_blocks);
    if (R <= 64) {
        for (int s = 0; s <= R; s++) first.push_back(seed_blocks + s);
        return;
    }
    for (int s = 0; s < 48; s++) first.push_back(seed_blocks + s);
    const int rem = R - 48;
    int64_t cum = 0;
    for (int k = 0; k < 16; k++) {
        first.push_back(seed_blocks + 48 + (int32_t)((int64_t)rem * cum / 136));
        cum += k + 1;
    }
    first.push_back(nblk);
    for (size_t k = 1; k < first.size(); k++) first[k] = std::max(first[k], first[k - 1]);
}

struct Plan {
    int c;
    int32_t Uc, sbase, pbase, Ic, a, b, CH, nch, q0, nq;
    int64_t ldm, B;
    bool pack24, prune, coop, half, panel;
    bool psym;
    bool flat;
    int32_t panel_cols, nsub;
    int64_t ldb64;
    int32_t tail_chunks, p_eff, tail_width;
    int32_t nblk;
    int64_t ldb;
};

#include "fy_rm2_coop.hpp"

static void validate_params(const fy_rm2_params* p) {
    if (!p) FY_FAIL(FY_ERR_INVALID_ARGUMENT, "params is NULL");
    if (p->number_of_clusters <= 0) FY_FAIL(FY_ERR_INVALID_ARGUMENT, "numberOfClusters must be > 0 (got %d)", p->number_of_clusters);
    if (p->number_of_items <= 0) FY_FAIL(FY_ERR_INVALID_ARGUMENT, "numberOfItems must be > 0 (got %d)", p->number_of_items);
    if (!(p->lambda >= 0.0 && p->lambda <= 1.0)) FY_FAIL(FY_ERR_INVALID_ARGUMENT, "lambda must be in [0, 1]");
    if (p->world <= 0 || p->rank < 0 || p->rank >= p->world) FY_FAIL(FY_ERR_INVALID_ARGUMENT, "rank %d of world %d", p->rank, p->world);
    if (p->number_of_recommendations < 0) FY_FAIL(FY_ERR_INVALID_ARGUMENT, "numberOfRecommendations must be >= 0");
}

static void build_tables_all(Context* ctx, const Prepared& P, const std::vector<Plan>& plans, const std::vector<int32_t>& csr_range, bool use_pk,
                             TableCache& tc, hipStream_t st) {
    const size_t np = plans.size();
    std::vector<CoDesc> hco(np);
    std::vector<SegDesc> hsd;
    std::vector<int64_t> main_of(np, -1), tail_of(np, -1);
    int64_t co_total = 0, co_tail_total = 0, cnt_total = 0;
    int32_t max_slots = 1, max_f = 1, max_nq = 1;
    for (size_t pi = 0; pi < np; pi++) {
        const Plan& p = plans[pi];
        const bool tail = p.p_eff < p.Ic;
        hco[pi] = CoDesc{p.sbase, p.Uc, p.CH, p.nch, csr_range[2 * pi], csr_range[2 * pi + 1], p.p_eff, tail ? 1 : 0, co_total, co_tail_total};
        SegDesc m{p.sbase, p.q0, p.nq, p.nch, p.CH, (p.half || p.psym) ? 1 : 0, 0, p.nch + 1, co_total, cnt_total, 0, p.psym ? p.p_eff : 0,
                  p.psym ? 0 : p.p_eff, (p.panel && p.tail_chunks > 0 && p.p_eff < p.Ic) ? p.tail_chunks : 0};
        main_of[pi] = (int64_t)hsd.size();
        hsd.push_back(m);
        cnt_total += (int64_t)p.nch * ((int64_t)p.nq + 1);
        co_total += (int64_t)p.Uc * (p.nch + 1);
        max_slots = std::max(max_slots, p.Uc);
        max_f = std::max(max_f, csr_range[2 * pi + 1] - csr_range[2 * pi]);
        max_nq = std::max(max_nq, p.nq);
    }
    for (size_t pi = 0; pi < np; pi++) {
        const Plan& p = plans[pi];
        if (p.p_eff >= p.Ic) continue;
        SegDesc t{p.sbase, p.q0, p.nq, 1, 0, 0, p.p_eff, 2, hco[pi].co_tail_off, cnt_total, 1, 0, 0, 0};
        tail_of[pi] = (int64_t)hsd.size();
        hsd.push_back(t);
        cnt_total += (int64_t)p.nq + 1;
    }
    for (size_t pi = 0; pi < np; pi++)
        if (plans[pi].p_eff < plans[pi].Ic) {  }
    {
        int64_t off = 0;
        for (size_t pi = 0; pi < np; pi++) {
            hco[pi].co_tail_off = off;
            if (plans[pi].p_eff < plans[pi].Ic) off += 2 * (int64_t)plans[pi].Uc;
        }
        co_tail_total = off;
        for (size_t pi = 0; pi < np; pi++)
            if (tail_of[pi] >= 0) hsd[(size_t)tail_of[pi]].co_off = hco[pi].co_tail_off;
    }
    if (cnt_total + 1 >= (int64_t)0x7FFFFFF0) FY_FAIL(FY_ERR_UNSUPPORTED, "segment tables of %zu clusters need %lld prefix entries (limit 2^31)", np, (long long)cnt_total);
    DevBuf<CoDesc> d_co(ctx, np);
    DevBuf<SegDesc> d_sd(ctx, hsd.size());
    FY_HIP(hipMemcpyAsync(d_co.get(), hco.data(), np * sizeof(CoDesc), hipMemcpyHostToDevice, st));
    FY_HIP(hipMemcpyAsync(d_sd.get(), hsd.data(), hsd.size() * sizeof(SegDesc), hipMemcpyHostToDevice, st));
    tc.g_co.alloc(ctx, (size_t)std::max<int64_t>(1, co_total));
    tc.g_co_tail.alloc(ctx, (size_t)std::max<int64_t>(1, co_tail_total));
    tc.g_cnt.alloc(ctx, (size_t)cnt_total + 1);
    tc.g_ptr.alloc(ctx, (size_t)cnt_total + 1);
    tc.g_start.alloc(ctx, (size_t)P.nnz + 1);
    const dim3 g_slots((unsigned)grid_for((int64_t)max_slots * 8, 256, 1024), (unsigned)np);
    if (use_pk) {
        k_pack_csr_multi<<<dim3((unsigned)grid_for(max_f, 256, 1024), (unsigned)np), 256, 0, st>>>(d_co.get(), P.csr_idx.get(), P.csr_r.get(), tc.csr_pk.get());
        FY_KERNEL_CHECK();
    }
    k_chunk_offsets_multi<<<g_slots, 256, 0, st>>>(d_co.get(), P.rowptr.get(), P.csr_idx.get(), tc.g_co.get());
    FY_KERNEL_CHECK();
    if (co_tail_total > 0) {
        k_tail_blocks_multi<<<dim3((unsigned)std::min<int>(max_slots, ctx->num_cus * 4), (unsigned)np), 256, 0, st>>>(d_co.get(), P.rowptr.get(), P.csr_idx.get(), P.csr_r.get(),
                                                                                                                  tc.y_pk.get(), tc.g_co_tail.get());
        FY_KERNEL_CHECK();
    }
    const unsigned n_main = (unsigned)np, n_tail = (unsigned)(hsd.size() - np);
    const dim3 g_q((unsigned)grid_for((int64_t)max_nq + 1, 256, 2048), n_main), g_qt((unsigned)grid_for((int64_t)max_nq + 1, 256, 2048), std::max(1u, n_tail));
    k_seg_counts_multi<<<g_q, 256, 0, st>>>(d_sd.get(), P.csc_slot.get(), tc.g_co.get(), tc.g_cnt.get(), tc.csc_rank.get(), P.csr_idx.get(), tc.g_start.get(), tc.samples.get());
    FY_KERNEL_CHECK();
    if (n_tail) {
        k_seg_counts_multi<<<g_qt, 256, 0, st>>>(d_sd.get() + np, P.csc_slot.get(), tc.g_co_tail.get(), tc.g_cnt.get(), tc.csc_rank.get(), P.csr_idx.get(), tc.g_start.get(), tc.samples.get());
        FY_KERNEL_CHECK();
    }
    FY_HIP(hipMemsetAsync(tc.g_cnt.get() + cnt_total, 0, sizeof(int32_t), st));
    exclusive_scan_i32(ctx, tc.g_cnt.get(), tc.g_ptr.get(), (size_t)cnt_total + 1, st);
    int32_t total = 0;
    FY_HIP(hipMemcpyAsync(&total, tc.g_ptr.get() + cnt_total, sizeof(int32_t), hipMemcpyDeviceToHost, st));
    FY_HIP(hipStreamSynchronize(st));
    tc.g_seg.alloc(ctx, (size_t)std::max(1, total));
    tc.g_w.alloc(ctx, (size_t)std::max(1, total));
    tc.total_segments = total;
    const float* csc_w = use_pk ? tc.csc_x_over_s.get() : tc.csc_x.get();
    const dim3 g_f((unsigned)grid_for((((int64_t)max_nq + 63) >> 6) * 64 * 4, 256, 4096), n_main), g_ft((unsigned)grid_for((((int64_t)max_nq + 63) >> 6) * 64, 256, 4096), std::max(1u, n_tail));
    k_seg_fill_multi<<<g_f, 256, 0, st>>>(d_sd.get(), P.csc_slot.get(), csc_w, tc.g_co.get(), tc.g_ptr.get(), tc.g_seg.get(), tc.g_w.get(), tc.csc_rank.get(),
                                          P.csr_idx.get(), tc.g_start.get());
    FY_KERNEL_CHECK();
    if (n_tail) {
        k_seg_fill_multi<<<g_ft, 256, 0, st>>>(d_sd.get() + np, P.csc_slot.get(), tc.csc_x_over_s.get(), tc.g_co_tail.get(), tc.g_ptr.get(), tc.g_seg.get(), tc.g_w.get(),
                                               tc.csc_rank.get(), P.csr_idx.get(), tc.g_start.get());
        FY_KERNEL_CHECK();
    }
    FY_HIP(hipStreamSynchronize(st));
    for (size_t pi = 0; pi < np; pi++) {
        SegTable& m = tc.segs[pi];
        m.v_ptr = tc.g_ptr.get() + hsd[(size_t)main_of[pi]].cnt_off;
        m.v_seg = tc.g_seg.get();
        m.v_w = tc.g_w.get();
        if (tail_of[pi] >= 0) {
            SegTable& t = tc.segs_tail[pi];
            t.v_ptr = tc.g_ptr.get() + hsd[(size_t)tail_of[pi]].cnt_off;
            t.v_seg = tc.g_seg.get();
            t.v_w = tc.g_w.get();
        }
    }
}

fy_rm2_job* fy::rm2_prepare(Context* ctx, const fy_rm2_params* prm, const fy_ratings* R, int64_t n_map, const int32_t* map_user,
                            const int32_t* map_cluster, const int32_t* cluster_count) {
    validate_params(prm);
    if (n_map < 0 || (n_map > 0 && (!map_user || !map_cluster))) FY_FAIL(FY_ERR_INVALID_ARGUMENT, "clustering map is NULL");
    EventTimer tm(ctx);
    const size_t span = tm.begin();
    const bool use_cache = !(prm->flags & FY_RM2_NO_CACHE);
    if (use_cache) {
        std::shared_ptr<RM2Static> have;
        {
            std::lock_guard<std::mutex> g(R->cache_mu);
            have = std::static_pointer_cast<RM2Static>(R->rm2_cache);
            if (have && !have->matches(prm, n_map, map_user, map_cluster, cluster_count)) { R->rm2_cache.reset(); have.reset(); }
        }
        if (have) {
            std::unique_ptr<fy_rm2_job> J(new fy_rm2_job(have));
            J->ctx = ctx;
            J->prm = *prm;
            J->from_cache = true;
            tm.end(span);
            sync(ctx);
            J->ms_prepare = tm.total_ms();
            return J.release();
        }
    }
    std::shared_ptr<RM2Static> fresh = std::make_shared<RM2Static>();
    fresh->K = prm->number_of_clusters;
    fresh->rank = prm->rank;
    fresh->world = prm->world;
    fresh->max_item = R->max_item;
    fresh->has_count = cluster_count != nullptr;
    if (n_map) { fresh->map_user.assign(map_user, map_user + n_map); fresh->map_cluster.assign(map_cluster, map_cluster + n_map); }
    if (cluster_count) fresh->cluster_count.assign(cluster_count, cluster_count + prm->number_of_clusters);
    std::unique_ptr<fy_rm2_job> J(new fy_rm2_job(fresh));
    J->ctx = ctx;
    J->prm = *prm;
    fy_ratings mine;
    DevBuf<int32_t> cl_table;
    SyncOnUnwind mine_guard(ctx->stream);
    RM2Static& S = *fresh;
    if (prm->world > 1 && ctx->tune.shard_prep)
        S.sharded = shard_ratings_by_cluster(ctx, R, prm->number_of_clusters, n_map, map_user, map_cluster, prm->rank, prm->world, mine, S.owner, cl_table);
    Prepared& P = J->P;
    if (S.sharded) {
        S.n_raw_users = (int64_t)R->max_user + 1;
        S.n_raw_items = (int64_t)R->max_item + 1;
        S.partial_raw.alloc(ctx, (size_t)S.exchange_len());
        S.partial_raw.zero();
        try {
            build_structure(ctx, &mine, prm->number_of_clusters, n_map, map_user, map_cluster, cluster_count, false, J->P, cl_table.get());
        } catch (const Failure& f) {
            if (f.code != FY_ERR_DUPLICATE_RATING && f.code != FY_ERR_CLUSTER_COUNT) throw;
            S.deferred_code = f.code;
            S.deferred_msg = last_error();
            const double flag = (double)(-f.code);
            sync(ctx);
            FY_HIP(hipMemcpyAsync(S.partial_raw.get() + (S.exchange_len() - 1), &flag, sizeof(double), hipMemcpyHostToDevice, ctx->stream));
            tm.end(span);
            sync(ctx);
            J->ms_prepare = tm.total_ms();
// ... 381 lines not shown
        }
        const int64_t flat_budget = tune.flat_budget > 0 ? tune.flat_budget : (int64_t)std::min<uint64_t>(ctx->total_mem / 4, (uint64_t)std::max<int64_t>(ws, (int64_t)8 << 30));
        auto flat_need = [](const Plan& p) {
            return (int64_t)p.Ic * p.ldm * (p.pack24 ? 3 : 4) + (int64_t)(p.b - p.a) * p.ldm * 4 + (int64_t)p.Ic * p.nch * 12 + 4096;
        };
        {
            int n_flat = 0;
            const bool can = tune.flat_batch && plans.size() > 1 && use_pk && tune.cooc_fx && !tune.cooc_f32 && !J->fx_bounds.empty() &&
                             prm.number_of_recommendations <= TOPN_LONG;
            for (auto& p : plans) {
                p.flat = false;
                if (!can || p.prune || p.coop || p.panel) continue;
                if (fx_exponent(&J->fx_bounds[3 * (size_t)p.c]) < 0) continue;
                if (flat_need(p) > flat_budget) continue;
                p.flat = true;
                n_flat++;
            }
            if (n_flat < 2)
                for (auto& p : plans) p.flat = false;
            for (auto& p : plans) p.psym = false;
            for (auto& p : plans)
                if (p.flat) p.half = false;
        }
        bool any_panel = false;
        for (auto& p : plans) any_panel = any_panel || p.panel;
        int64_t panel_bytes = 0;
        int n_panel = 0;
        for (auto& p : plans)
            if (p.panel) { n_panel++; panel_bytes += (int64_t)p.Ic * p.panel_cols * 3 + (int64_t)p.Ic * p.ldb64 * 7 + 64; }
        const bool two_phase = tune.panel_two_phase && n_panel >= 2;
        std::vector<int> group_of(plans.size(), 0);
        int n_groups = 1;
        if (two_phase) {
            const int64_t limit = tune.panel_group_bytes > 0 ? tune.panel_group_bytes : (int64_t)(ctx->total_mem / 3);
            int64_t in_group = 0;
            int g = 0;
            for (size_t pi = 0; pi < plans.size(); pi++) {
                const Plan& p = plans[pi];
                if (!p.panel) continue;
                const int64_t need = (int64_t)p.Ic * p.panel_cols * 3 + (int64_t)p.Ic * p.ldb64 * 7 + (int64_t)(p.b - p.a) * p.ldb64 * 7 + (int64_t)p.Ic * p.nch * 12;
                if (in_group > 0 && in_group + need > limit) { g++; in_group = 0; }
                in_group += need;
                group_of[pi] = g;
            }
            n_groups = g + 1;
        }
        (void)panel_bytes;
        if (two_phase && tune.panel_sym && tune.panel_multi_launch && use_pk && tune.cooc_fx && !tune.cooc_f32 && !J->fx_bounds.empty())
            for (auto& p : plans)
                p.psym = p.panel && p.tail_chunks > 0 && p.p_eff < p.Ic && p.p_eff == p.panel_cols && p.p_eff % 256 == 0 && p.a == p.sbase && p.b == p.sbase + p.Uc &&
                         fx_exponent(&J->fx_bounds[3 * (size_t)p.c]) >= 0;
        const int want_lanes = tune.lanes_forced ? tune.lanes : (two_phase ? std::max(tune.lanes, 8) : (any_panel ? std::min(tune.lanes, tune.panel_lanes) : tune.lanes));
        const int NS = (int)std::min<size_t>(plans.size() > 1 ? (size_t)want_lanes : 1, plans.size());
        if (!(NS == 1 && plans.size() == 1 && !plans[0].coop && !plans[0].flat && !plans[0].panel)) join_values(st);
        struct Lane {
            hipStream_t st;
            DevBuf<float> M, S;
            DevBuf<int32_t> overflow, any_overflow;
            DevBuf<float> Bmax, amax, bmax, UB, tau;
            DevBuf<float> Gp, Bmax64, amax64, bmax64;
            DevBuf<uint32_t> Brep;
            DevBuf<uint16_t> surv;
            DevBuf<uint8_t> surv_mask;
            DevBuf<int2> strayT;
            DevBuf<int2> stray_items;
            DevBuf<int32_t> n_heavy;
            DevBuf<int32_t> need;
            DevBuf<float> Bsup, asup, bsupb, UBs;
            DevBuf<double> head32, tail32;
            DevBuf<int32_t> colmap;
            DevBuf<int32_t> sup_first;
            DevBuf<int32_t> n_quads, quad_prefix;
            DevBuf<char> scan_tmp;
            DevBuf<int2> item_seg, item_seg_t;
            DevBuf<int32_t> item_id, item_id_t;
            DevBuf<float> Ssurv;
        };
        std::vector<Lane> lanes((size_t)NS);
        {
            size_t is_el = 1;
            for (auto& p : plans)
                if (!p.flat) is_el = std::max(is_el, (size_t)p.Ic * p.nch);
            size_t m_el = 1, s_el = 1, ov_el = 1, bm_el = 1, ub_el = 1, am_el = 1, gp_el = 1, b64_el = 1, a64_el = 1;
            for (auto& p : plans) {
                p.B = std::min<int64_t>(std::max<int64_t>(1, (ws / NS) / (p.ldm * 4)), p.b - p.a);
                const int64_t seed_cols = (int64_t)std::min<int64_t>(ceil_div(p.Ic, 256), tune.seed_chunks) * 256;
                if (p.prune || p.flat) p.B = p.b - p.a;
                if (p.coop || p.flat) continue;
                if (p.panel) {
                    gp_el = std::max(gp_el, (size_t)p.Ic * p.panel_cols * 3 / 4 + 4);
                    b64_el = std::max(b64_el, (size_t)p.Ic * p.ldb64 * 3 / 4 + 4);
                    a64_el = std::max(a64_el, (size_t)p.ldb64);

                    s_el = std::max(s_el, (size_t)(p.B * seed_cols));
                    ov_el = std::max(ov_el, (size_t)p.B);
                    ub_el = std::max(ub_el, (size_t)(p.B * p.ldb64));
                    continue;
                }
                m_el = std::max(m_el, (size_t)(p.Ic * p.ldm));
                s_el = std::max(s_el, (size_t)(p.B * (p.prune ? seed_cols : p.ldm)));
                ov_el = std::max(ov_el, (size_t)p.B);
                if (p.prune) {
                    bm_el = std::max(bm_el, (size_t)(p.Ic * p.ldb));
                    ub_el = std::max(ub_el, (size_t)(p.B * p.ldb));
                    am_el = std::max(am_el, (size_t)p.ldb);
                }
            }
            if (NS > 1 && ctx->aux.size() < (size_t)NS) {
                while (ctx->aux.size() < (size_t)NS) {
                    hipStream_t x;
                    FY_HIP(hipStreamCreateWithFlags(&x, hipStreamNonBlocking));
                    ctx->aux.push_back(x);
                }
            }
            for (int l = 0; l < NS; l++) {
                Lane& L = lanes[l];
                L.st = NS > 1 ? ctx->aux[l] : st;
                L.M.alloc(ctx, m_el);
                L.S.alloc(ctx, s_el);
                L.overflow.alloc(ctx, ov_el);
                L.any_overflow.alloc(ctx, 1);
                L.n_heavy.alloc(ctx, 1);
                L.Bmax.alloc(ctx, bm_el);
                L.amax.alloc(ctx, am_el);
                L.bmax.alloc(ctx, am_el);
                L.Gp.alloc(ctx, two_phase ? 1 : gp_el);
                L.Bmax64.alloc(ctx, two_phase ? 1 : b64_el);
                L.Brep.alloc(ctx, gp_el > 1 && !two_phase ? b64_el * 4 / 3 + 4 : 1);
                L.amax64.alloc(ctx, two_phase ? 1 : a64_el);
                L.bmax64.alloc(ctx, two_phase ? 1 : a64_el);
                L.UB.alloc(ctx, ub_el);
                L.tau.alloc(ctx, ov_el);
                L.surv.alloc(ctx, ub_el);
                L.surv_mask.alloc(ctx, gp_el > 1 ? ub_el : 1);
                L.n_quads.alloc(ctx, ov_el + 1);
                L.quad_prefix.alloc(ctx, ov_el + 1);
                L.item_seg.alloc(ctx, is_el);
                L.item_id.alloc(ctx, is_el);
            }
        }
        DevBuf<unsigned long long> prune_counters(ctx, 6);
        prune_counters.zero();
        int64_t prune_blocks_total = 0, prune_seed_terms_cols = 0, coop_survived = 0, fallback_survived = 0;
        for (auto& p : plans) any_coop = any_coop || p.coop;
        bool any_tail = false, any_half = false;
        size_t co_all = 1;
        for (auto& p : plans) {
            any_tail = any_tail || p.p_eff < p.Ic;
            co_all = std::max(co_all, (size_t)p.Uc * (p.nch + 1));
            any_half = any_half || p.half || p.p_eff < p.Ic;
        }
        std::vector<int32_t> sig;
        sig.push_back(use_pk ? 1 : 0);
        sig.push_back(plans.size() > 1 && !any_coop ? 1 : 0);
        for (auto& p : plans) {
            const int32_t v[8] = {p.c, p.CH, p.nch, p.half ? 1 : 0, p.panel ? 1 : 0, p.p_eff, p.tail_chunks, (p.coop ? 1 : 0) | (p.flat ? 2 : 0) | (p.psym ? 4 : 0)};
            sig.insert(sig.end(), v, v + 8);
        }
        const bool tables_cached = tc.valid && tc.sig == sig;
        R->st.tables_from_cache = tables_cached ? 1 : 0;
        span_tables = t_tables.begin();
        if (!tables_cached) {
            tc.valid = false;
            segs.clear();
            segs_tail.clear();
            segs.resize(plans.size());
            segs_tail.resize(plans.size());
            csr_pk.alloc(ctx, use_pk ? (size_t)P.nnz : 1);
            y_pk.alloc(ctx, any_tail ? (size_t)P.nnz : 1);
            csc_rank.alloc(ctx, any_half ? (size_t)P.nnz : 1);
            if (any_half) {
                k_csc_rank<<<grid_for(P.nnz), 256, 0, st>>>(P.nnz, P.csc_pair.get(), P.pair_rank.get(), csc_rank.get());
                FY_KERNEL_CHECK();
                build_csr_samples(ctx, P.nnz, P.csr_idx.get(), tc.samples, st);
            }
        }
        std::vector<int32_t> csr_range(2 * plans.size() + 2, 0);
        {
            std::vector<int32_t> where(2 * plans.size());
            for (size_t pi = 0; pi < plans.size(); pi++) {
                where[2 * pi] = plans[pi].sbase;
                where[2 * pi + 1] = plans[pi].sbase + plans[pi].Uc;
            }
            gather_to_host_i32(ctx, P.rowptr.get(), where, csr_range.data());
        }
        const bool bounded_tables = false;
        auto build_tables = [&](size_t pi, hipStream_t ts, int32_t* co) {
            if (tables_cached) return;
            const Plan& p = plans[pi];
            const int32_t f0 = csr_range[2 * pi], f1 = csr_range[2 * pi + 1];
            if (use_pk && f1 > f0) {
                k_pack_csr<<<grid_for(f1 - f0), 256, 0, ts>>>(f0, f1, p.CH, P.csr_idx.get(), P.csr_r.get(), csr_pk.get());
                FY_KERNEL_CHECK();
            }
            if (p.coop) return;
            build_chunk_offsets(ctx, P.rowptr.get(), P.csr_idx.get(), p.sbase, p.Uc, p.CH, p.nch, co, ts);
            const int64_t deg2_c = (size_t)p.c < P.cluster_deg2.size() ? P.cluster_deg2[p.c] : 0;
            const int64_t seg_bound = bounded_tables && deg2_c > 0 ? deg2_c / 64 + (int64_t)p.nq * p.nch + 64 : 0;
            build_segments(ctx, P.csc_slot.get(), use_pk ? csc_x_over_s.get() : csc_x.get(), co, p.sbase, p.q0, p.nq, p.nch, segs[pi], ts,
                           p.half ? csc_rank.get() : nullptr, P.csr_idx.get(), p.CH, nullptr, 0, seg_bound, p.half ? tc.samples.get() : nullptr);
            if (p.p_eff < p.Ic) {
                k_tail_blocks<<<std::min<int>(p.Uc, ctx->num_cus * 16), 256, 0, ts>>>(p.sbase, p.Uc, p.p_eff, P.rowptr.get(), P.csr_idx.get(), P.csr_r.get(),
                                                                          y_pk.get(), co);
                FY_KERNEL_CHECK();
                build_segments(ctx, P.csc_slot.get(), csc_x_over_s.get(), co, p.sbase, p.q0, p.nq, 1, segs_tail[pi], ts, nullptr, nullptr, 0,
                               csc_rank.get(), p.p_eff, bounded_tables && deg2_c > 0 ? deg2_c / 64 + (int64_t)p.nq + 64 : 0);
            }
        };
        const bool all_at_once = plans.size() > 1 && !any_coop;
        const bool lazy_tables = false;
        std::vector<DevBuf<int32_t>> co_lane((size_t)NS);
        if (!all_at_once)
            for (auto& b : co_lane) b.alloc(ctx, co_all);
        if (all_at_once) {
            if (!tables_cached) build_tables_all(ctx, P, plans, csr_range, use_pk, tc, st);
        } else if (!lazy_tables)
            for (size_t pi = 0; pi < plans.size(); pi++) build_tables(pi, st, co_lane[0].get());
        t_tables.end(span_tables);
        DevBuf<char> flatM;
        DevBuf<float> flatS;
        DevBuf<int2> flat_seg;
        DevBuf<int32_t> flat_id, flat_ov, flat_flags, flat_cnt;
        DevBuf<CoocLaunch> d_flat_launch;
        DevBuf<FlatDesc> d_flat[2];
        for (size_t first = 0; first < plans.size();) {
            std::vector<CoocLaunch> fb;
            std::vector<FlatDesc> fd[2];
            SyncOnUnwind fb_fd_guard(st);
            size_t m_bytes = 0, s_el = 0, i_el = 0, u_el = 0, n_flat = 0, last = first;
            int64_t batch_bytes = 0;
            for (; last < plans.size(); last++) {
                const Plan& p = plans[last];
                if (!p.flat) continue;
                if (n_flat && batch_bytes + flat_need(p) > flat_budget) break;
                batch_bytes += flat_need(p);
                m_bytes += round_up((int64_t)p.Ic * p.ldm * (p.pack24 ? 3 : 4), 256);
                s_el += (size_t)(p.b - p.a) * p.ldm;
                i_el += (size_t)p.Ic * p.nch;
                u_el += (size_t)(p.b - p.a);
                n_flat++;
            }
            if (n_flat) {
                flatM.alloc(ctx, m_bytes);
                flatS.alloc(ctx, s_el);
                flat_seg.alloc(ctx, i_el);
                flat_id.alloc(ctx, i_el);
                flat_ov.alloc(ctx, u_el);
                flat_flags.alloc(ctx, 2 * n_flat);
                size_t m_at = 0, s_at = 0, i_at = 0, u_at = 0, k = 0;
                int max_grid[2] = {0, 0}, max_users[2] = {0, 0};
                for (size_t pi = first; pi < last; pi++) {
                    const Plan& p = plans[pi];
                    if (!p.flat) continue;
                    const int c = p.c;
                    const int32_t nb = p.b - p.a;
                    float* const Mc = reinterpret_cast<float*>(flatM.get() + m_at);
                    float* const Sc = flatS.get() + s_at;
                    CoocArgs CA{P.rank_pair.get(), P.pair_start.get(), segs[pi].ptr_(), segs[pi].seg_(), segs[pi].w_(), P.csr_idx.get(),
                                csr_x.get(), p.pbase, p.sbase, p.Ic, p.CH, p.nch, 0, p.Ic, p.q0, p.nq, nullptr, 0, csr_pk.get(), nullptr,
                                (uint32_t)std::min<int64_t>((int64_t)P.nnz * 4, 0xFFFFFFFFll)};
                    const int fxk = fx_exponent(&J->fx_bounds[3 * (size_t)c]);
                    CA.fx_scale = std::ldexp(1.0, fxk);
                    const double w2s = (1.0 - lambda) * (1.0 - lambda) * (double)h_gscale[(size_t)c];
                    MEpilogue ME{Mc, p.ldm, (float)w2s, std::ldexp(w2s, -fxk), p.pack24 ? 1 : 0, nullptr, p.ldb, 0, 0, nullptr, p.ldb64, nullptr};
                    const int n_items = (int)cooc_item_count(p.Ic, p.CH, p.nch, false);
                    CA.item_seg = flat_seg.get() + i_at;
                    CA.item_id = flat_id.get() + i_at;
                    CA.item_grab = cooc_item_grab((size_t)c < P.cluster_deg2.size() ? P.cluster_deg2[c] : P.sum_deg2, n_items);
                    fb.push_back(CoocLaunch{CA, ME, n_items, 0});

                    const int n_chunks = (int)ceil_div(p.Ic, 64 * VEC);
                    const int64_t fill = ceil_div(8 * (int64_t)ctx->num_cus, (int64_t)std::max(1, n_chunks) * (int64_t)n_flat);
                    const int n_slices = (int)std::max<int64_t>(1, std::min<int64_t>(tune.max_slices, std::min<int64_t>(ceil_div(nb, 4), std::max<int64_t>(ceil_div(nb, 4 * (int64_t)tune.users_per_wave), fill))));
                    FlatDesc d{};
                    ScoreArgs& SA = d.SA;
                    SA.M = Mc; SA.ldm = p.ldm; SA.Ic = p.Ic; SA.a_rank = a_rank.get() + p.pbase; SA.b_rank = b_rank32.get() + p.pbase;
                    SA.rb_off = P.rowptr.get() + p.sbase;
                    SA.csr_idx = P.csr_idx.get(); SA.csr_e = csr_e.get(); SA.csr_q = csr_q.get();
                    SA.pvpi = pvpi.get(); SA.n_out = n_out.get(); SA.slot_lo = lo; SA.slot_base = p.sbase; SA.slot0 = p.a; SA.n_users = nb;
                    SA.S = Sc; SA.ldS = p.ldm; SA.n_slices = n_slices; SA.n_chunks = n_chunks;
                    d.n_heavy = flat_flags.get() + 2 * k;
                    d.any_overflow = flat_flags.get() + 2 * k + 1;
                    SA.n_heavy = tune.score_heavy > 0 ? d.n_heavy : nullptr;
                    d.heavy_thresh = tune.score_heavy > 0 ? std::min(tune.score_heavy, 32) : 0x7FFFFFFF;
                    d.TA = TopNArgs{Sc, p.ldm, p.Ic, n_out.get(), out_off.get(), P.rank_item_raw.get() + p.pbase, P.slot2du.get(), P.uid.get(), lo, p.a, c,
                                    R->d_key0.get(), R->d_key1.get(), R->d_value.get(), R->d_aux.get(), 0, 0, nullptr, nullptr, 0, nullptr, nullptr, nullptr};
                    d.overflow = flat_ov.get() + u_at;
                    d.score_grid = n_chunks * n_slices;
                    d.n_users = nb;
                    const int f = p.pack24 ? 1 : 0;
                    max_grid[f] = std::max(max_grid[f], d.score_grid);
                    max_users[f] = std::max(max_users[f], nb);
                    fd[f].push_back(d);
                    m_at += (size_t)round_up((int64_t)p.Ic * p.ldm * (p.pack24 ? 3 : 4), 256);
                    s_at += (size_t)nb * p.ldm;
                    i_at += (size_t)p.Ic * p.nch;
                    u_at += (size_t)nb;
                    k++;
                }
                const size_t sp = t_cooc.begin(st);
                launch_cooc_rm2_multi(ctx, tune, fb, false, d_flat_launch, flat_cnt, st, true);
                t_cooc.end(sp, st);
                R->st.cooc_launches++;
                for (int f = 0; f < 2; f++) {
                    if (fd[f].empty()) continue;
                    const unsigned ny = (unsigned)fd[f].size();
                    d_flat[f].alloc(ctx, fd[f].size());
                    FY_HIP(hipMemcpyAsync(d_flat[f].get(), fd[f].data(), fd[f].size() * sizeof(FlatDesc), hipMemcpyHostToDevice, st));
                    const size_t ss = t_score.begin(st);
                    k_count_heavy_multi<<<(ny + 63) / 64, 64, 0, st>>>(d_flat[f].get(), (int32_t)ny);
                    FY_KERNEL_CHECK();
                    if (f) k_score_multi<4, true, 8><<<dim3((unsigned)max_grid[f], ny), 256, 0, st>>>(d_flat[f].get(), P.csr_idx.get(), csr_e.get(), csr_q.get(), pvpi.get(), n_out.get());
                    else k_score_multi<4, false, 8><<<dim3((unsigned)max_grid[f], ny), 256, 0, st>>>(d_flat[f].get(), P.csr_idx.get(), csr_e.get(), csr_q.get(), pvpi.get(), n_out.get());
                    FY_KERNEL_CHECK();
                    t_score.end(ss, st);
                    R->st.score_launches++;
                    const size_t tt = t_topn.begin(st);
                    k_topn_fast_multi<<<dim3((unsigned)max_users[f], ny), 256, 0, st>>>(d_flat[f].get(), tune.force_select);
                    FY_KERNEL_CHECK();
                    k_topn_select_multi<<<dim3((unsigned)max_users[f], ny), 256, 0, st>>>(d_flat[f].get(), prune_counters.get() + 2);
                    FY_KERNEL_CHECK();
                    t_topn.end(tt, st);
                }
                FY_HIP(hipStreamSynchronize(st));
            }
            first = last;
        }
        struct PanelBuf {
            DevBuf<float> Gp, Bmax64, amax64, bmax64;
            DevBuf<uint32_t> Brep;
            DevBuf<double> head32, tail32;
        };
        struct PanelPtrs {
            float *Gp, *Bmax64;
            uint32_t* Brep;
            float *amax64, *bmax64;
        };
        std::vector<PanelBuf> pbuf(two_phase ? plans.size() : 0);
        std::vector<Lane> plane(two_phase ? plans.size() : 0);
        auto group_buffers = [&](int grp) {
            for (size_t pi = 0; pi < plans.size(); pi++) {
                const Plan& p = plans[pi];
                if (!p.panel || group_of[pi] != grp) continue;
                pbuf[pi].Gp.alloc(ctx, (size_t)p.Ic * p.panel_cols * 3 / 4 + 4);
                pbuf[pi].Bmax64.alloc(ctx, (size_t)p.Ic * p.ldb64 * 3 / 4 + 4);
                pbuf[pi].Brep.alloc(ctx, (size_t)p.Ic * p.ldb64 + 4);
                pbuf[pi].amax64.alloc(ctx, (size_t)p.ldb64);
                pbuf[pi].bmax64.alloc(ctx, (size_t)p.ldb64);
            }
            for (size_t pi = 0; pi < plans.size(); pi++) {
                const Plan& p = plans[pi];
                if (!p.panel || group_of[pi] != grp) continue;
                Lane& W = plane[pi];
                const size_t nbp = (size_t)(p.b - p.a);
                const size_t seed_cols = (size_t)std::min<int64_t>(ceil_div(p.Ic, 256), tune.seed_chunks) * 256;
                W.st = lanes[pi % NS].st;
                W.M.alloc(ctx, 1); W.Bmax.alloc(ctx, 1); W.amax.alloc(ctx, 1); W.bmax.alloc(ctx, 1);
                W.Gp.alloc(ctx, 1); W.Bmax64.alloc(ctx, 1); W.Brep.alloc(ctx, 1); W.amax64.alloc(ctx, 1); W.bmax64.alloc(ctx, 1);
                W.item_seg.alloc(ctx, (size_t)p.Ic * p.nch); W.item_id.alloc(ctx, (size_t)p.Ic * p.nch);
                W.item_seg_t.alloc(ctx, (size_t)std::max(1, p.Ic - p.p_eff)); W.item_id_t.alloc(ctx, (size_t)std::max(1, p.Ic - p.p_eff));
                W.S.alloc(ctx, nbp * seed_cols);
                W.overflow.alloc(ctx, nbp);
                W.any_overflow.alloc(ctx, 1);
                W.n_heavy.alloc(ctx, 1);
                W.UB.alloc(ctx, nbp * (size_t)p.ldb64);
                W.tau.alloc(ctx, nbp);
                W.surv.alloc(ctx, nbp * (size_t)p.ldb64);
                W.surv_mask.alloc(ctx, nbp * (size_t)p.ldb64);
                W.n_quads.alloc(ctx, nbp + 1);
                W.quad_prefix.alloc(ctx, nbp + 1);
            }
        };
        std::vector<CoocLaunch> batch_main, batch_tail;
        DevBuf<CoocLaunch> d_batch_main, d_batch_tail;
        DevBuf<int32_t> d_cnt_main, d_cnt_tail;
        DevBuf<PanelDesc> d_panel_desc;
        std::vector<PanelDesc> hpd;
        struct LaneGuard {
            Context* ctx;
            hipEvent_t fork = nullptr;
            int32_t* pinned = nullptr;
            ~LaneGuard() {
                for (hipStream_t x : ctx->aux) (void)hipStreamSynchronize(x);
                (void)hipStreamSynchronize(ctx->stream);
                if (fork) (void)hipEventDestroy(fork);
                if (pinned) (void)hipHostFree(pinned);
            }
        } guard{ctx};
        if (two_phase) FY_HIP(hipHostMalloc(reinterpret_cast<void**>(&guard.pinned), plans.size() * sizeof(int32_t), hipHostMallocDefault));
        for (int grp = 0; grp < n_groups; grp++) {
        if (two_phase) {
            if (grp > 0) {
                for (size_t pi = 0; pi < plans.size(); pi++)
                    if (plans[pi].panel && group_of[pi] == grp - 1) { pbuf[pi] = PanelBuf(); plane[pi] = Lane(); }
            }
            group_buffers(grp);
            batch_main.clear();
            batch_tail.clear();
            hpd.clear();
        }
        for (int phase = two_phase ? 1 : 0; phase <= (two_phase ? 3 : 0); phase++) {
        const auto host_t0 = std::chrono::steady_clock::now();
        struct PhaseClock {
            const std::chrono::steady_clock::time_point t0;
            int grp, phase;
            bool on;
            ~PhaseClock() {
                if (on) fprintf(stderr, "[fy] group %d phase %d: host queued for %.3f ms\n", grp, phase, std::chrono::duration<double, std::milli>(std::chrono::steady_clock::now() - t0).count());
            }
        } phase_clock{host_t0, grp, phase, tune.debug_sync != 0};
        if (phase == 3) {
            for (int l = 0; l < NS; l++) FY_HIP(hipStreamSynchronize(lanes[l].st));
            FY_HIP(hipStreamSynchronize(st));
        }
        if ((phase == 0 || phase == 2) && NS > 1) {
            if (guard.fork) { FY_HIP(hipEventDestroy(guard.fork)); guard.fork = nullptr; }
            FY_HIP(hipEventCreateWithFlags(&guard.fork, hipEventDisableTiming));
            FY_HIP(hipEventRecord(guard.fork, st));
            for (int l = 0; l < NS; l++) FY_HIP(hipStreamWaitEvent(lanes[l].st, guard.fork, 0));
        }

        for (size_t pi = 0; pi < plans.size(); pi++) {
            const Plan& p = plans[pi];
            if (p.flat) continue;
            if (group_of[pi] != grp) continue;
            if ((phase == 1 || phase == 3) && !p.panel) continue;
            Lane& L = phase == 1 ? lanes[0] : (two_phase && p.panel ? plane[pi] : lanes[pi % NS]);
            hipStream_t ls = phase == 1 ? st : L.st;
            const bool do_build = !(phase >= 2 && p.panel), do_score = phase != 1;
            const PanelPtrs PP = two_phase && p.panel ? PanelPtrs{pbuf[pi].Gp.get(), pbuf[pi].Bmax64.get(), pbuf[pi].Brep.get(), pbuf[pi].amax64.get(), pbuf[pi].bmax64.get()}
                                                      : PanelPtrs{L.Gp.get(), L.Bmax64.get(), L.Brep.get(), L.amax64.get(), L.bmax64.get()};
            auto checkpoint = [&](const char* what) {
                if (tune.debug_sync != 1) return;
                const hipError_t e = hipDeviceSynchronize();
                fprintf(stderr, "[fy] group %d/%d phase %d plan %zu (cluster %d): %s -> %s\n", grp, n_groups, phase, pi, p.c, what, hipGetErrorString(e));
                fflush(stderr);
            };
            checkpoint("start");
            if (p.panel && (!PP.Gp || !PP.Bmax64 || !PP.Brep || !PP.amax64 || !PP.bmax64 || (two_phase && (!L.S.get() || !L.UB.get() || !L.n_quads.get()) && phase != 1)))
                FY_FAIL(FY_ERR_STATE, "internal: cluster %d (plan %zu, group %d of %d, phase %d) has no panel buffers", p.c, pi, grp, n_groups, phase);
            const int c = p.c;
            const int32_t sbase = p.sbase, pbase = p.pbase, Ic = p.Ic, a = p.a, b = p.b, CH = p.CH, nch = p.nch;
            const int64_t ldm = p.ldm;
            const bool pack24 = p.pack24;
            if (p.coop) {
                CoopShared X{J, R.get(), &tune, b_rank32.get(), a_rank.get(), use_pk ? csc_x_over_s.get() : csc_x.get(), csr_x.get(), csr_e.get(), csr_q.get(),
                             use_pk ? csr_pk.get() : nullptr,
                             n_out.get(), out_off.get(), pvpi.get(), lo, &t_cooc, &t_score, &t_topn, prune_counters.get(),
                             &prune_blocks_total, &prune_seed_terms_cols, &coop_survived, &coop_pair_contribs, d_cshift.get(), h_gscale[(size_t)c]};
                score_cluster_coop(X, p, ls);
                continue;
            }

            if (lazy_tables) {
                const size_t stb = t_tables.begin(ls);
                build_tables(pi, ls, co_lane[pi % NS].get());
                t_tables.end(stb, ls);
            }
            CoocArgs CA{P.rank_pair.get(), P.pair_start.get(), segs[pi].ptr_(), segs[pi].seg_(), segs[pi].w_(), P.csr_idx.get(),
                        csr_x.get(), pbase, sbase, Ic, CH, nch, 0, Ic, p.q0, p.nq, nullptr, 0, use_pk ? csr_pk.get() : nullptr, nullptr,
                        (uint32_t)std::min<int64_t>((int64_t)P.nnz * 4, 0xFFFFFFFFll)};
            const int fxk = (use_pk && tune.cooc_fx && !J->fx_bounds.empty()) ? fx_exponent(&J->fx_bounds[3 * (size_t)c]) : -1;
            CA.fx_scale = fxk >= 0 ? std::ldexp(1.0, fxk) : 0.0;
            const double w2s = (1.0 - lambda) * (1.0 - lambda) * (double)h_gscale[(size_t)c];
            MEpilogue ME{L.M.get(), ldm, (float)w2s, fxk >= 0 ? std::ldexp(w2s, -fxk) : 0.0,
                         pack24 ? 1 : 0, (p.prune && !p.panel) ? L.Bmax.get() : nullptr, p.ldb, 0,
                         p.panel ? p.panel_cols : 0, p.panel ? PP.Bmax64 : nullptr, p.ldb64, p.panel ? PP.Brep : nullptr};
            if (p.panel) ME.M = PP.Gp;
            const bool refine = tune.refine && pack24 && !p.coop && fxk >= 0 && J->S->max_item >= 0 && J->S->max_item < (1 << 28) && Ic >= 8;
            const int32_t head_rows = (int32_t)std::min<int64_t>(Ic & ~3, std::max<int64_t>(256, std::min<int64_t>(1024, (int64_t)tune.seed_chunks * 256)));
            const int64_t ld_head = p.psym ? (int64_t)p.p_eff : ldm;
            DevBuf<double>& H32 = (two_phase && p.panel) ? pbuf[pi].head32 : L.head32;
            DevBuf<double>& T32 = (two_phase && p.panel) ? pbuf[pi].tail32 : L.tail32;
            if (refine && do_build) {
                H32.alloc(ctx, (size_t)head_rows * ld_head + 4);
                if (p.psym) T32.alloc(ctx, (size_t)std::max(1, Ic - p.p_eff) * head_rows + 4);
                ME.head32 = H32.get();
                ME.ld_head = ld_head;
                ME.head_rows = head_rows;
                ME.tail32 = p.psym ? T32.get() : nullptr;
                ME.tail_from = p.p_eff;
            }
            if (do_build) {
            if (p.panel) {
                R->st.panel_clusters++;
                FY_HIP(hipMemsetAsync(PP.Bmax64, 0, (size_t)Ic * p.ldb64 * 3, ls));
                k_block_amax<<<grid_for(p.ldb64), 256, 0, ls>>>(Ic, (int32_t)p.ldb64, a_rank.get() + pbase, b_rank32.get() + pbase, PP.amax64,
                                                               PP.bmax64, 64);
                FY_KERNEL_CHECK();
            } else if (p.prune) {
                FY_HIP(hipMemsetAsync(L.Bmax.get(), 0, (size_t)Ic * p.ldb * 3, ls));
                k_block_amax<<<grid_for(p.ldb), 256, 0, ls>>>(Ic, (int32_t)p.ldb, a_rank.get() + pbase, b_rank32.get() + pbase, L.amax.get(), L.bmax.get());
                FY_KERNEL_CHECK();
            }
            const size_t sp = t_cooc.begin(ls);
            const bool batched = phase == 1 && tune.panel_multi_launch && use_pk && fxk >= 0 && !tune.cooc_f32;
            if (p.p_eff < Ic) {
                CoocArgs CB{P.rank_pair.get(), P.pair_start.get(), segs_tail[pi].ptr_(), segs_tail[pi].seg_(), segs_tail[pi].w_(), P.csr_idx.get(),
                            csr_x.get(), pbase, sbase, Ic, p.tail_width, 1, p.p_eff, Ic - p.p_eff, p.q0, p.nq, nullptr, 0, y_pk.get(), nullptr, CA.pk_bytes};
                CB.fx_scale = CA.fx_scale;
                MEpilogue MB{reinterpret_cast<float*>(reinterpret_cast<char*>(PP.Bmax64) + (size_t)(p.p_eff / 64) * 3), p.tail_width, ME.w2, ME.fx_inv, 1,
                             nullptr, 0, 0, 0, nullptr, 0, nullptr, p.ldb64, 1};
                int2* const tseg = batched ? plane[pi].item_seg_t.get() : L.item_seg.get();
                int32_t* const tid = batched ? plane[pi].item_id_t.get() : L.item_id.get();
                if (!batched) {
                    k_item_list<<<grid_for((int64_t)(Ic - p.p_eff)), 256, 0, ls>>>(CB, tseg, tid);
                    FY_KERNEL_CHECK();
                }
                CB.item_seg = tseg;
                CB.item_id = tid;
                CB.item_grab = 8;
                if (batched) batch_tail.push_back(CoocLaunch{CB, MB, Ic - p.p_eff, 0});
                else {
                    FY_HIP(hipMemsetAsync(L.any_overflow.get(), 0, sizeof(int32_t), ls));
                    launch_cooc_rm2(ctx, tune, use_pk, CB, MB, Ic - p.p_eff, L.any_overflow.get(), ls);
                    R->st.cooc_launches++;
                }
                CA.tail_row0 = p.p_eff;
                CA.tail_chunks = p.tail_chunks;
            }
            {
                CA.half = (p.half || p.psym) ? 1 : 0;
                if (p.psym) { CA.half_rows = p.p_eff; CA.head_chunks = p.tail_chunks; }
                const int n_items = p.psym ? (int)(cooc_half_item_index(p.p_eff - 1, p.tail_chunks - 1, CH, p.tail_chunks) + 1 + (int64_t)(Ic - p.p_eff) * p.tail_chunks)
                                    : CA.tail_chunks > 0 ? (int)((int64_t)p.p_eff * nch + (int64_t)(Ic - p.p_eff) * p.tail_chunks)
                                                         : (int)cooc_item_count(Ic, CH, nch, p.half);
                int2* const mseg = batched ? plane[pi].item_seg.get() : L.item_seg.get();
                int32_t* const mid = batched ? plane[pi].item_id.get() : L.item_id.get();
                if (!batched) {
                    k_item_list<<<grid_for((int64_t)Ic * nch), 256, 0, ls>>>(CA, mseg, mid);
                    FY_KERNEL_CHECK();
                }
                CA.item_seg = mseg;
                CA.item_id = mid;
                CA.item_grab = cooc_item_grab(((size_t)c < P.cluster_deg2.size() ? P.cluster_deg2[c] : P.sum_deg2) / (p.half ? 2 : 1), n_items);
                if (batched) batch_main.push_back(CoocLaunch{CA, ME, n_items, 0});
                else {
                    FY_HIP(hipMemsetAsync(L.any_overflow.get(), 0, sizeof(int32_t), ls));
                    launch_cooc_rm2(ctx, tune, use_pk, CA, ME, n_items, L.any_overflow.get(), ls);
                }
            }
            t_cooc.end(sp, ls);
            join_values(ls);
            checkpoint("row kernel queued / run");
            if (!batched) R->st.cooc_launches++;
            if (p.half) {
                const size_t sm = t_mirror.begin(ls);
                const bool lazy = p.prune && tune.lazy_mirror;
                launch_mirror(ctx, L.M.get(), ldm, Ic, p.prune ? L.Bmax.get() : nullptr, p.ldb, ls, nullptr, lazy ? std::min(tune.seed_chunks, p.nblk) : 0x7FFFFFFF);
                t_mirror.end(sm, ls);
            }
            if (p.prune && !p.panel && tune.sup_bounds && !long_seed) {
                const int seed_b = std::min(tune.seed_chunks, p.nblk);
                std::vector<int32_t> first;
                sup_block_map(seed_b, p.nblk, first);
                const int n_sup = (int)first.size() - 1;
                first.resize(65, first.back());
                L.sup_first.alloc(ctx, 65);
                L.Bsup.alloc(ctx, (size_t)Ic * 64);
                L.asup.alloc(ctx, 64);
                L.bsupb.alloc(ctx, 64);
                FY_HIP(hipMemcpyAsync(L.sup_first.get(), first.data(), 65 * sizeof(int32_t), hipMemcpyHostToDevice, ls));
                FY_HIP(hipStreamSynchronize(ls));
                const size_t sb = t_score.begin(ls);
                k_build_bsup<<<std::min<int>((Ic + 3) / 4, ctx->num_cus * 32), 256, 0, ls>>>(Ic, n_sup, L.sup_first.get(), L.Bmax.get(), p.ldb, L.Bsup.get());
                FY_KERNEL_CHECK();
                k_sup_amax<<<1, 64, 0, ls>>>(n_sup, L.sup_first.get(), L.amax.get(), L.bmax.get(), L.asup.get(), L.bsupb.get());
                FY_KERNEL_CHECK();
                t_score.end(sb, ls);
            }
            }
            if (!do_score) continue;

            const int64_t ldS = ldm, B = p.B;
            const int n_chunks = (int)ceil_div(Ic, 64 * VEC);
            const int32_t* row_off = P.rowptr.get() + sbase;
            auto score_args = [&](const float* Mx, int64_t ldmx, int32_t Icx, const float* ax, int32_t s0, int32_t nb, float* Sx, int64_t ldSx,
                                  int n_slices, int nchunks) {
                ScoreArgs SA{};
                SA.M = Mx; SA.ldm = ldmx; SA.Ic = Icx; SA.a_rank = ax; SA.b_rank = b_rank32.get() + pbase; SA.rb_off = row_off;
                SA.csr_idx = P.csr_idx.get(); SA.csr_e = csr_e.get(); SA.csr_q = csr_q.get();
                SA.pvpi = pvpi.get(); SA.n_out = n_out.get(); SA.slot_lo = lo; SA.slot_base = sbase; SA.slot0 = s0; SA.n_users = nb;
                SA.S = Sx; SA.ldS = ldSx; SA.n_slices = n_slices; SA.n_chunks = nchunks;
                if (tune.score_heavy > 0) {
                    const int heavy = (int64_t)nb * nchunks < 8 * (int64_t)ctx->num_cus ? std::min(tune.score_heavy, 32) : tune.score_heavy;
                    k_count_heavy<<<1, 64, 0, ls>>>(P.rowptr.get() + s0, nb, heavy, L.n_heavy.get());
                    SA.n_heavy = L.n_heavy.get();
                }
                return SA;
            };
            auto refine_rows = [&](int32_t s0, int32_t nb) {
                if (!refine || nb <= 0) return;
                const size_t tt = t_topn.begin(ls);
                const int32_t n_ids = J->S->max_item + 1;
                L.colmap.alloc(ctx, (size_t)n_ids);
                FY_HIP(hipMemsetAsync(L.colmap.get(), 0xFF, (size_t)n_ids * sizeof(int32_t), ls));
                k_refine_colmap<<<(head_rows + 255) / 256, 256, 0, ls>>>(head_rows, P.rank_item_raw.get() + pbase, L.colmap.get());
                FY_KERNEL_CHECK();
                RefineArgs RA{};
                RA.slot0 = s0; RA.n_users = nb; RA.slot_lo = lo; RA.slot_base = sbase;
                RA.n_out = n_out.get(); RA.out_off = out_off.get(); RA.out_item = R->d_key1.get(); RA.out_score = R->d_value.get(); RA.out_item_w = R->d_key1.get();
                RA.rowptr = P.rowptr.get(); RA.csr_idx = P.csr_idx.get(); RA.csr_r = P.csr_r.get(); RA.usum_slot = J->usum_slot.get();
                RA.p_rank = p_rank.get() + pbase; RA.b_rank = b_rank.get() + pbase;
                RA.colmap = L.colmap.get(); RA.max_item = J->S->max_item;
                RA.head_rows = head_rows;
                RA.head32 = H32.get(); RA.ld_head = ld_head; RA.tail32 = p.psym ? T32.get() : nullptr; RA.tail_from = p.p_eff;
                if (!RA.head32 || (p.psym && !RA.tail32)) FY_FAIL(FY_ERR_STATE, "internal: cluster %d has no fp32 rows for the refinement pass", c);
                RA.unscale = 1.0 / (double)h_gscale[(size_t)c];
                RA.lambda = lambda; RA.ln_items = std::log((double)prm.number_of_items); RA.ln_users = std::log((double)p.Uc);
                RA.users_minus_1 = (double)(p.Uc - 1);
                RA.refine_c = tune.refine_c;
                RA.n_refined = prune_counters.get() + 5;
                int lp2 = 64;
                while (lp2 < std::min<int>(prm.number_of_recommendations, Ic)) lp2 <<= 1;
                k_refine_rows<<<(nb + 3) / 4, 256, (size_t)4 * lp2 * sizeof(uint64_t), ls>>>(RA);
                FY_KERNEL_CHECK();
                t_topn.end(tt, ls);
            };
            auto full_pass = [&](int32_t s0, int32_t nb, float* Sx) {
                const int n_slices = score_slices(ctx, tune, nb, n_chunks);
                ScoreArgs SA = score_args(L.M.get(), ldm, Ic, a_rank.get() + pbase, s0, nb, Sx, ldS, n_slices, n_chunks);
                const size_t ss = t_score.begin(ls);
                if (pack24) k_score<4, true, 8><<<n_chunks * n_slices, 256, 0, ls>>>(SA.M, SA.a_rank, SA.rb_off, SA.csr_idx, SA.csr_e, SA.csr_q, SA.pvpi, SA.n_out, SA.S, SA);
                else k_score<4, false, 8><<<n_chunks * n_slices, 256, 0, ls>>>(SA.M, SA.a_rank, SA.rb_off, SA.csr_idx, SA.csr_e, SA.csr_q, SA.pvpi, SA.n_out, SA.S, SA);
                FY_KERNEL_CHECK();
                t_score.end(ss, ls);
                R->st.score_launches++;
                TopNArgs TA{Sx, ldS, Ic, n_out.get(), out_off.get(), P.rank_item_raw.get() + pbase, P.slot2du.get(), P.uid.get(), lo, s0, c,
                            R->d_key0.get(), R->d_key1.get(), R->d_value.get(), R->d_aux.get(), 0, 0, nullptr, nullptr, 0, nullptr, nullptr, nullptr};
                const size_t tt = t_topn.begin(ls);
                FY_HIP(hipMemsetAsync(L.any_overflow.get(), 0, sizeof(int32_t), ls));
                if (prm.number_of_recommendations > TOPN_LONG)
                    k_topn_long<<<nb, 256, (size_t)fy_topn_long_cap(prm.number_of_recommendations) * 8, ls>>>(TA, L.overflow.get(), L.any_overflow.get(), tune.force_select,
                                                                                                         fy_topn_long_cap(prm.number_of_recommendations));
                else k_topn_fast<<<nb, 256, 0, ls>>>(TA, L.overflow.get(), L.any_overflow.get(), tune.force_select);
                FY_KERNEL_CHECK();
                k_topn_select<<<nb, 256, 0, ls>>>(TA, L.overflow.get(), L.any_overflow.get(), prune_counters.get() + 2);
                FY_KERNEL_CHECK();
                t_topn.end(tt, ls);
                refine_rows(s0, nb);
            };
            for (int32_t s0 = a; s0 < b; s0 += (int32_t)B) {
                const int32_t nb = (int32_t)std::min<int64_t>(B, b - s0);
                if (!p.prune) { full_pass(s0, nb, L.S.get()); continue; }
                const int seed_chunks = std::min(n_chunks, tune.seed_chunks);
                const bool use_sup = tune.sup_bounds && !p.panel && !long_seed;
                const int n_slices = score_slices(ctx, tune, nb, seed_chunks + (use_sup ? 0 : (int)(p.ldb / 256)));
                const bool split = two_phase && p.panel && s0 == sbase && nb == p.Uc;
                if (phase == 3 && !split) continue;
                size_t ss = t_score.begin(ls);
                const int seed_blocks = seed_chunks;
                const int64_t SC = (int64_t)seed_chunks * 256;
                const float* Gmat = p.panel ? PP.Gp : L.M.get();
// ... 333 lines not shown
```

### filmyou-core_amd/csrc/fy_rm2_coop.hpp

```cpp
#pragma once

struct CoopShared {
    fy_rm2_job* J;
    fy_result* R;
    const ScoreTune* tune;
    const float *b_rank;
    const float *a_rank, *csc_x, *csr_x, *csr_e, *csr_q;
    const uint32_t* csr_pk;
    const int32_t *n_out, *out_off;
    const double* pvpi;
    int32_t lo;
    EventTimer *t_cooc, *t_score, *t_topn;
    unsigned long long* prune_counters;
    int64_t *blocks_total, *seed_terms_cols, *coop_survived, *coop_pair_contribs;
    const int32_t* cshift;
    float gscale;
};

static void coll_all_gather(fy_rm2_job* J, const void* send, void* recv, int64_t bytes, hipStream_t st) {
    if (!J->have_coll) {
        if (bytes) FY_HIP(hipMemcpyAsync(recv, send, (size_t)bytes, hipMemcpyDeviceToDevice, st));
        return;
    }
    const int rc = J->coll.all_gather(J->coll.user, send, recv, bytes, (void*)st);
    if (rc) FY_FAIL(FY_ERR_COLLECTIVE, "all_gather callback returned %d", rc);
}
static void coll_reduce_scatter(fy_rm2_job* J, const float* send, float* recv, int64_t count, hipStream_t st) {
    if (!J->have_coll) {
        if (count) FY_HIP(hipMemcpyAsync(recv, send, (size_t)count * sizeof(float), hipMemcpyDeviceToDevice, st));
        return;
    }
    const int rc = J->coll.reduce_scatter_f32(J->coll.user, send, recv, count, (void*)st);
    if (rc) FY_FAIL(FY_ERR_COLLECTIVE, "reduce_scatter callback returned %d", rc);
}

static void score_cluster_coop(const CoopShared& X, const Plan& p, hipStream_t ls) {
    fy_rm2_job* J = X.J;
    Context* ctx = J->ctx;
    Prepared& P = J->P;
    fy_result* R = X.R;
    const ScoreTune& tune = *X.tune;
    const fy_rm2_params& prm = J->prm;
    const int W = prm.world, me = prm.rank;
    const int32_t Uc = p.Uc, sbase = p.sbase, pbase = p.pbase, Ic = p.Ic, CH = p.CH, nch = p.nch;
    const int64_t ldm = p.ldm, ldb = p.ldb;
    const double lambda = prm.lambda;

    std::vector<int32_t> ua(W), ub(W);
    int32_t Umax = 1;
    for (int k = 0; k < W; k++) {
        int32_t lo_k, hi_k;
        owner_range(J, k, lo_k, hi_k);
        ua[k] = std::max(lo_k, sbase);
        ub[k] = std::max(ua[k], std::min(hi_k, sbase + Uc));
        Umax = std::max(Umax, ub[k] - ua[k]);
    }
    const int32_t my_a = ua[me], n_mine = ub[me] - ua[me];

    const int32_t r0 = me, nrows = Ic > me ? (Ic - me + W - 1) / W : 0;
    std::vector<int32_t> hcnt((size_t)Ic);
    int64_t my_ratings = 0, my_walk = 0;
    {
        std::vector<long long> hw((size_t)Ic);
        FY_HIP(hipMemcpyAsync(hw.data(), J->walk_rank.get() + pbase, (size_t)Ic * sizeof(long long), hipMemcpyDeviceToHost, ls));
        FY_HIP(hipMemcpyAsync(hcnt.data(), J->cnt_rank.get() + pbase, (size_t)Ic * sizeof(int32_t), hipMemcpyDeviceToHost, ls));
        FY_HIP(hipStreamSynchronize(ls));
        for (int32_t i = r0; i < Ic; i += W) { my_ratings += hcnt[i]; my_walk += hw[i]; }
    }
    *X.coop_pair_contribs += my_walk - my_ratings;

    const int n_chunks = (int)ceil_div(Ic, 256);
    const int seed_chunks = std::min(n_chunks, tune.seed_chunks);
    const int seed_blocks = seed_chunks;
    const int64_t SC = (int64_t)seed_chunks * 256;
    const int bchunks = (int)(ldb / 256);
    DevBuf<float> Mloc(ctx, (size_t)std::max<int64_t>(1, (int64_t)nrows * ldm * 3 / 4 + 4)), Bloc(ctx, (size_t)std::max<int64_t>(1, (int64_t)nrows * ldb));
    DevBuf<float> amax(ctx, (size_t)ldb), bmax(ctx, (size_t)ldb);
    DevBuf<int32_t> n_out_all(ctx, (size_t)Uc), item_counter(ctx, 1);
    const int64_t nnz_c = (int64_t)p.nq;
    DevBuf<int32_t> my_cnt(ctx, (size_t)Uc + 1), my_rowptr(ctx, (size_t)Uc + 1), my_idx(ctx, (size_t)std::max<int64_t>(1, nnz_c));
    DevBuf<float> my_e(ctx, (size_t)std::max<int64_t>(1, nnz_c)), my_q(ctx, (size_t)std::max<int64_t>(1, nnz_c));
    DevBuf<double> pv_all(ctx, (size_t)Uc);
    DevBuf<unsigned long long> dummy(ctx, 2);
    DevBuf<float> seed_send(ctx, (size_t)((int64_t)W * Umax * SC)), seed(ctx, (size_t)((int64_t)Umax * SC));
    DevBuf<float> ub_send(ctx, (size_t)((int64_t)W * Umax * ldb)), UBsum(ctx, (size_t)((int64_t)Umax * ldb));
    DevBuf<float> tau(ctx, (size_t)Umax);
    DevBuf<uint16_t> surv(ctx, (size_t)((int64_t)Umax * ldb));
    DevBuf<int32_t> n_quads(ctx, (size_t)Umax + 1), quad_prefix(ctx, (size_t)Umax + 1), overflow(ctx, (size_t)Umax), any_overflow(ctx, 1);
    DevBuf<int32_t> counts(ctx, (size_t)W);
    const float* Mshift = Mloc.get();
    const float* Bshift = Bloc.get();

    {
        DevBuf<int32_t> co_tmp(ctx, (size_t)Uc * (nch + 1));
        SegTable seg;
        DevBuf<int2> item_seg(ctx, (size_t)std::max<int64_t>(1, (int64_t)nrows * nch));
        DevBuf<int32_t> item_id(ctx, (size_t)std::max<int64_t>(1, (int64_t)nrows * nch));
        build_chunk_offsets(ctx, P.rowptr.get(), P.csr_idx.get(), sbase, Uc, CH, nch, co_tmp.get(), ls);
        std::vector<int32_t> hls((size_t)nrows + 1, 0);
        for (int32_t i = 0; i < nrows; i++) hls[i + 1] = hls[i] + hcnt[r0 + (int64_t)i * W];
        DevBuf<int32_t> local_start(ctx, (size_t)nrows + 1), my_slot(ctx, (size_t)std::max<int64_t>(1, my_ratings));
        DevBuf<float> my_w(ctx, (size_t)std::max<int64_t>(1, my_ratings));
        FY_HIP(hipMemcpyAsync(local_start.get(), hls.data(), ((size_t)nrows + 1) * sizeof(int32_t), hipMemcpyHostToDevice, ls));
        if (nrows > 0) {
            k_gather_rows<<<grid_for((int64_t)nrows * 64, 256), 256, 0, ls>>>(r0, W, nrows, P.rank_pair.get() + pbase, P.pair_start.get(),
                                                                              local_start.get(), P.csc_slot.get(), X.csc_x, my_slot.get(), my_w.get());
            FY_KERNEL_CHECK();
        }
        build_segments(ctx, my_slot.get(), my_w.get(), co_tmp.get(), sbase, 0, (int32_t)my_ratings, nch, seg, ls);
        FY_HIP(hipMemsetAsync(Bloc.get(), 0, (size_t)std::max<int64_t>(1, (int64_t)nrows * ldb) * 3, ls));
        k_block_amax<<<grid_for(ldb), 256, 0, ls>>>(Ic, (int32_t)ldb, X.a_rank + pbase, X.b_rank + pbase, amax.get(), bmax.get());
        FY_KERNEL_CHECK();
        if (nrows > 0) {
            CoocArgs CA{P.rank_pair.get(), P.pair_start.get(), seg.ptr.get(), seg.seg.get(), seg.w.get(), P.csr_idx.get(),
                        X.csr_x, pbase, sbase, Ic, CH, nch, r0, nrows, 0, (int32_t)my_ratings, local_start.get(), W, X.csr_pk, nullptr,
                        (uint32_t)std::min<int64_t>((int64_t)P.nnz * 4, 0xFFFFFFFFll)};
            const int fxk = (X.csr_pk && tune.cooc_fx && !J->fx_bounds.empty()) ? fx_exponent(&J->fx_bounds[3 * (size_t)p.c]) : -1;
            CA.fx_scale = fxk >= 0 ? std::ldexp(1.0, fxk) : 0.0;
            const double w2s = (1.0 - lambda) * (1.0 - lambda) * (double)X.gscale;
            MEpilogue ME{const_cast<float*>(Mshift), ldm, (float)w2s, fxk >= 0 ? std::ldexp(w2s, -fxk) : 0.0,
                         1, const_cast<float*>(Bshift), ldb, 1};
            const size_t sp = X.t_cooc->begin(ls);
            const int n_items = nrows * nch;
            k_item_list<<<grid_for(n_items), 256, 0, ls>>>(CA, item_seg.get(), item_id.get());
            FY_KERNEL_CHECK();
            CA.item_seg = item_seg.get();
            CA.item_id = item_id.get();
            FY_HIP(hipMemsetAsync(item_counter.get(), 0, sizeof(int32_t), ls));
            launch_cooc_rm2(ctx, tune, X.csr_pk != nullptr, CA, ME, n_items, item_counter.get(), ls);
            X.t_cooc->end(sp, ls);
            R->st.cooc_launches++;
        }
        FY_HIP(hipStreamSynchronize(ls));
    }

    k_my_csr_count<<<grid_for(((int64_t)Uc + 1) * 64, 256), 256, 0, ls>>>(Uc, sbase, P.rowptr.get(), P.csr_idx.get(), W, me, my_cnt.get());
    FY_KERNEL_CHECK();
    exclusive_scan_i32(ctx, my_cnt.get(), my_rowptr.get(), (size_t)Uc + 1, ls);
    k_my_csr_fill<<<grid_for((int64_t)Uc * 64, 256), 256, 0, ls>>>(Uc, sbase, P.rowptr.get(), P.csr_idx.get(), X.csr_e, X.csr_q, W, me, my_rowptr.get(),
                                                                   my_idx.get(), my_e.get(), my_q.get());
    FY_KERNEL_CHECK();
    FY_HIP(hipMemsetAsync(dummy.get(), 0, 2 * sizeof(unsigned long long), ls));
    k_user_meta<<<grid_for(Uc), 256, 0, ls>>>(sbase, sbase + Uc, P.slot2du.get(), P.uid.get(), P.ucluster.get(), P.udeg.get(),
                                               P.d_csize.get(), P.d_pcstart.get(), prm.number_of_items, prm.number_of_recommendations,
                                               prm.filter_users, X.cshift, pv_all.get(), n_out_all.get(), dummy.get());
    FY_KERNEL_CHECK();
    if (me != 0) FY_HIP(hipMemsetAsync(pv_all.get(), 0, (size_t)Uc * sizeof(double), ls));

    size_t ss = X.t_score->begin(ls);
    auto slices_for = [&](int32_t nb) { return score_slices(ctx, tune, nb, seed_chunks + bchunks); };
    for (int k = 0; k < W; k++) {
        const int32_t nk = ub[k] - ua[k];
        if (nk <= 0) continue;
        const int ns = slices_for(nk);
        ScoreArgs SA{};
        SA.M = Mshift; SA.ldm = ldm; SA.Ic = Ic; SA.a_rank = X.a_rank + pbase; SA.b_rank = X.b_rank + pbase; SA.rb_off = my_rowptr.get();
        SA.csr_idx = my_idx.get(); SA.csr_e = my_e.get(); SA.csr_q = my_q.get(); SA.pvpi = pv_all.get(); SA.n_out = n_out_all.get(); SA.slot_lo = sbase; SA.slot_base = sbase; SA.slot0 = ua[k];
        SA.n_users = nk; SA.S = seed_send.get() + (int64_t)k * Umax * SC; SA.ldS = SC; SA.n_slices = ns; SA.n_chunks = seed_chunks + bchunks;
        SA.row_mul = W; SA.row_add = me;
        SA.chunks1 = seed_chunks;
        SA.M2 = Bshift;
        SA.ldm2 = ldb;
        SA.Ic2 = p.nblk;
        SA.a2 = amax.get();
        SA.b2 = bmax.get();
        SA.S2 = ub_send.get() + (int64_t)k * Umax * ldb;
        SA.ldS2 = ldb;
        SA.no_mask2 = 1;
        k_score<4, true, 8><<<(seed_chunks + bchunks) * ns, 256, 0, ls>>>(SA.M, SA.a_rank, SA.rb_off, SA.csr_idx, SA.csr_e, SA.csr_q, SA.pvpi, SA.n_out, SA.S, SA);
        FY_KERNEL_CHECK();
        R->st.score_launches += 2;
    }
    X.t_score->end(ss, ls);
    coll_reduce_scatter(J, seed_send.get(), seed.get(), (int64_t)Umax * SC, ls);
    coll_reduce_scatter(J, ub_send.get(), UBsum.get(), (int64_t)Umax * ldb, ls);
    ss = X.t_score->begin(ls);
    if (n_mine > 0) {
        TopNArgs T1{seed.get(), SC, Ic, X.n_out, X.out_off, P.rank_item_raw.get() + pbase, P.slot2du.get(), P.uid.get(),
                    X.lo, my_a, p.c, R->d_key0.get(), R->d_key1.get(), R->d_value.get(), R->d_aux.get(),
                    1, (int32_t)SC, surv.get(), n_quads.get(), ldb, tau.get(), nullptr, nullptr};
        k_topn_fast<<<n_mine, 256, 0, ls>>>(T1, overflow.get(), any_overflow.get(), 0);
        FY_KERNEL_CHECK();
    }
    FY_HIP(hipMemsetAsync(n_quads.get(), 0, ((size_t)Umax + 1) * sizeof(int32_t), ls));
    if (n_mine > 0) {
        k_bound_select<<<grid_for((int64_t)n_mine * 64, 256), 256, 0, ls>>>(UBsum.get(), ldb, p.nblk, seed_blocks, tau.get(), X.pvpi + (my_a - X.lo), n_mine,
                                                                            surv.get(), n_quads.get());
        FY_KERNEL_CHECK();
    }
    exclusive_scan_i32(ctx, n_quads.get(), quad_prefix.get(), (size_t)n_mine + 1, ls);
    DevBuf<int32_t> my_count(ctx, 1);
    FY_HIP(hipMemcpyAsync(my_count.get(), quad_prefix.get() + n_mine, sizeof(int32_t), hipMemcpyDeviceToDevice, ls));
    X.t_score->end(ss, ls);
    coll_all_gather(J, my_count.get(), counts.get(), sizeof(int32_t), ls);
    ss = X.t_score->begin(ls);
    std::vector<int32_t> hcounts((size_t)W);
    FY_HIP(hipMemcpyAsync(hcounts.data(), counts.get(), (size_t)W * sizeof(int32_t), hipMemcpyDeviceToHost, ls));
    FY_HIP(hipStreamSynchronize(ls));
    int32_t t_max = 0;
    for (int k = 0; k < W; k++) t_max = std::max(t_max, hcounts[k]);
    DevBuf<float> Ssurv;
    if (t_max > 0) {
        DevBuf<long long> entries(ctx, (size_t)t_max), entries_all(ctx, (size_t)W * t_max);
        DevBuf<float> Spart(ctx, (size_t)W * t_max * PRUNE_BLOCK);
        Ssurv.alloc(ctx, (size_t)t_max * PRUNE_BLOCK);
        FY_HIP(hipMemsetAsync(entries.get(), 0, (size_t)t_max * sizeof(long long), ls));
        if (n_mine > 0) {
            k_surv_entries<<<grid_for((int64_t)n_mine * 64, 256), 256, 0, ls>>>(n_mine, my_a, quad_prefix.get(), surv.get(), ldb, entries.get());
            FY_KERNEL_CHECK();
        }
        X.t_score->end(ss, ls);
        coll_all_gather(J, entries.get(), entries_all.get(), (int64_t)t_max * (int64_t)sizeof(long long), ls);
        ss = X.t_score->begin(ls);
        k_score_entries<8><<<ctx->num_cus * 8, 256, 0, ls>>>(Mshift, X.a_rank + pbase, X.b_rank + pbase, my_rowptr.get(), my_idx.get(), my_e.get(), my_q.get(), pv_all.get(),
                                                             entries_all.get(), counts.get(), W, t_max, sbase, Ic, ldm, W, me, Spart.get(),
                                                             X.prune_counters);
        FY_KERNEL_CHECK();
        R->st.score_launches++;
        X.t_score->end(ss, ls);
        coll_reduce_scatter(J, Spart.get(), Ssurv.get(), (int64_t)t_max * PRUNE_BLOCK, ls);
        ss = X.t_score->begin(ls);
        FY_HIP(hipStreamSynchronize(ls));
    }
    X.t_score->end(ss, ls);
    if (n_mine > 0 && hcounts[me] > 0) {
        const size_t tt = X.t_topn->begin(ls);
        TopNArgs TA{seed.get(), SC, Ic, X.n_out, X.out_off, P.rank_item_raw.get() + pbase, P.slot2du.get(), P.uid.get(),
                    X.lo, my_a, p.c, R->d_key0.get(), R->d_key1.get(), R->d_value.get(), R->d_aux.get(),
                    2, (int32_t)SC, surv.get(), n_quads.get(), ldb, tau.get(), Ssurv.get(), quad_prefix.get()};
        FY_HIP(hipMemsetAsync(any_overflow.get(), 0, sizeof(int32_t), ls));
        k_topn_fast<<<n_mine, 256, 0, ls>>>(TA, overflow.get(), any_overflow.get(), tune.force_select);
        FY_KERNEL_CHECK();
        k_topn_select<<<n_mine, 256, 0, ls>>>(TA, overflow.get(), any_overflow.get(), X.prune_counters + 2);
        FY_KERNEL_CHECK();
        X.t_topn->end(tt, ls);
    }
    *X.blocks_total += (int64_t)n_mine * std::max(0, p.nblk - seed_blocks);
    *X.coop_survived += (int64_t)hcounts[me];
    *X.seed_terms_cols += my_ratings * (SC + ldb);
    FY_HIP(hipStreamSynchronize(ls));
}
```

Measured before the change: 403.1 million.

## Pre-permute packed CSR column index to LDS plane layout and drop per-element masking

The packed CSR and tail-block words now store the accumulator index already mapped into the quartered LDS plane layout, so the row kernel's inner commit loop computes the LDS byte address with a single SDWA shift instead of a mask/multiply/shift sequence. The per-lane row-cut compare is replaced by a wave-uniform OWN template path that removes the single owning lane from an exec mask via ballot, and atomics go through explicit LDS address-space pointers. The pack layout is recorded in the kernel arguments and checked at launch, and the planes flag is added to the cache signature. This trims ALU work in the hottest accumulation loop, at the cost of a second kernel instantiation and extra ballots per element on cut rows.

```diff
diff --git a/filmyou-core_amd/csrc/fy_cooc.hpp b/filmyou-core_amd/csrc/fy_cooc.hpp
--- a/filmyou-core_amd/csrc/fy_cooc.hpp
+++ b/filmyou-core_amd/csrc/fy_cooc.hpp
@@ -37,9 +37,10 @@
     int32_t acc_quarter;
     int32_t acc32;
     int32_t half_rows, head_chunks;
+    int32_t pk_layout;
 };
 __device__ __forceinline__ bool cooc_row_is_cut(const CoocArgs& A, int row) { return A.half && (A.half_rows == 0 || row < A.half_rows); }
-__device__ __forceinline__ int cooc_acc_index(int c, int quarter) { return quarter ? (c & 3) * quarter + (c >> 2) : c; }
+__host__ __device__ __forceinline__ int cooc_acc_index(int c, int quarter) { return quarter ? (c & 3) * quarter + (c >> 2) : c; }
 
 #ifndef FY_COOC_NB
 #define FY_COOC_NB 8
@@ -151,9 +152,8 @@
 __device__ __forceinline__ __amdgpu_buffer_rsrc_t cooc_pk_rsrc(const CoocArgs& A) {
     return __builtin_amdgcn_make_buffer_rsrc(const_cast<uint32_t*>(A.csr_pk), 0, (int)A.pk_bytes, 0x00020000);
 }
-template <class ACC>
-__device__ __forceinline__ void cooc_accumulate_pk(const CoocArgs& A, ACC* __restrict__ acc, int s_begin, int s_end, SegBatch first,
-                                                   int rmask = -1 ) {
+template <class ACC, bool OWN>
+__device__ __forceinline__ void cooc_accumulate_pk(const CoocArgs& A, ACC* __restrict__ acc, int s_begin, int s_end, SegBatch first, int own_word = 0) {
     const int lane = threadIdx.x & 63;
     const int wave = __builtin_amdgcn_readfirstlane(threadIdx.x >> 6);
     const int nwaves = blockDim.x >> 6;
@@ -161,29 +161,40 @@
     const int lane4 = lane * 4;
     constexpr int NB = FY_COOC_NB;
     using Group = PkGroup;
-    auto issue = [&](Group& G, const int2& d, float w, int g) __attribute__((always_inline)) { cooc_pk_issue(rsrc, lane4, G, d, w, g); };
     const double fx = A.fx_scale;
-    const uint32_t ix_mask = A.acc_quarter ? 3u : 0u, ix_shift = A.acc_quarter ? 2u : 0u, ix_quarter = (uint32_t)A.acc_quarter;
+    const uint32_t own = (uint32_t)__builtin_amdgcn_readfirstlane(own_word);
+    const int acc_shift = sizeof(ACC) == 8 ? 3 : 2;
+    typedef __attribute__((address_space(3))) char* lds_bytes;
+    typedef __attribute__((address_space(3))) ACC* lds_acc;
+    const lds_bytes acc_base = (lds_bytes)acc;
     auto commit = [&](Group& G) __attribute__((always_inline)) {
 #pragma unroll
         for (int q = 0; q < NB; q++) {
             const float x = __half2float(__ushort_as_half((unsigned short)(G.pk[q] >> 16)));
+            uint32_t at;
+            asm volatile("v_lshlrev_b32_sdwa %0, %1, %2 dst_sel:DWORD dst_unused:UNUSED_PAD src0_sel:DWORD src1_sel:WORD_0" : "=v"(at) : "s"(acc_shift), "v"(G.pk[q]));
+            unsigned long long m = __ballot(lane < G.L[q]);
+            if constexpr (OWN) {
+                const unsigned long long hit = __ballot(at == own * (uint32_t)sizeof(ACC)) & m;
+                if (hit) m &= ~1ull << (63 - __builtin_clzll(hit));
+            }
             if constexpr (std::is_same<ACC, uint32_t>::value) {
-                const uint32_t v = (uint32_t)(G.W[q] * x * (float)fx);
-                if (lane < G.L[q] && (int)(G.pk[q] & 0xFFFFu) > rmask) atomicAdd(&acc[cooc_acc_index((int)(G.pk[q] & 0xFFFFu), A.acc_quarter)], v);
+                uint32_t v = (uint32_t)(G.W[q] * x * (float)fx);
+                asm volatile("" : "+v"(v));
+                if (__builtin_amdgcn_inverse_ballot_w64(m)) __hip_atomic_fetch_add((lds_acc)(acc_base + at), v, __ATOMIC_RELAXED, __HIP_MEMORY_SCOPE_AGENT);
             } else if constexpr (std::is_same<ACC, unsigned long long>::value) {
                 const double d = fma((double)(G.W[q] * x), fx, 4503599627370496.0);
                 unsigned long long v = (unsigned long long)__double_as_longlong(d) & 0xFFFFFFFFFFFFFull;
-                const uint32_t c = G.pk[q] & 0xFFFFu;
-                uint32_t at = __umul24(c & ix_mask, ix_quarter) + (c >> ix_shift);
-                asm volatile("" : "+v"(at), "+v"(v));
-                if (lane < G.L[q] && (int)c > rmask) atomicAdd(&acc[at], v);
+                asm volatile("" : "+v"(v));
+                if (__builtin_amdgcn_inverse_ballot_w64(m)) __hip_atomic_fetch_add((lds_acc)(acc_base + at), v, __ATOMIC_RELAXED, __HIP_MEMORY_SCOPE_AGENT);
             } else {
-                const ACC v = (ACC)(G.W[q] * x);
-                if (lane < G.L[q] && (int)(G.pk[q] & 0xFFFFu) > rmask) atomicAdd(&acc[cooc_acc_index((int)(G.pk[q] & 0xFFFFu), A.acc_quarter)], v);
+                ACC v = (ACC)(G.W[q] * x);
+                asm volatile("" : "+v"(v));
+                if (__builtin_amdgcn_inverse_ballot_w64(m)) __hip_atomic_fetch_add((lds_acc)(acc_base + at), v, __ATOMIC_RELAXED, __HIP_MEMORY_SCOPE_AGENT);
             }
         }
     };
+    auto issue = [&](Group& G, const int2& d, float w, int g) __attribute__((always_inline)) { cooc_pk_issue(rsrc, lane4, G, d, w, g); };
     int batch = 0;
     if (cooc_seg_slot(s_begin, 0, wave, nwaves, 0) >= s_end) return;
     int2 d = first.d;
@@ -226,7 +237,7 @@
         s_begin = sp[e0];
         s_end = sp[e1];
     }
-    if constexpr (PK) cooc_accumulate_pk<double>(A, fy_cooc_acc, s_begin, s_end, cooc_first_batch(A, s_begin, s_end));
+    if constexpr (PK) cooc_accumulate_pk<double, false>(A, fy_cooc_acc, s_begin, s_end, cooc_first_batch(A, s_begin, s_end));
     else cooc_accumulate_segments<false, double>(A, fy_cooc_acc, s_begin, s_end, ch * A.CH, cooc_first_batch(A, s_begin, s_end));
 }
 
@@ -309,6 +320,7 @@
                          int32_t CH, int32_t nch, int32_t* chunk_off, hipStream_t st = nullptr);
 
 __host__ __device__ inline int cooc_lds_columns(int CH) { return (CH % 256 == 0) ? CH : ((CH + 255) / 256) * 256 + 256; }
+__host__ __device__ inline int cooc_acc_quarter(bool planes, int CH) { return planes ? cooc_lds_columns(CH) / 4 : 0; }
 
 inline void pick_chunks(int32_t Ic, int32_t max_ch, int32_t& CH, int32_t& nch) {
     if (Ic <= max_ch) {
diff --git a/filmyou-core_amd/csrc/fy_rm2.hip b/filmyou-core_amd/csrc/fy_rm2.hip
--- a/filmyou-core_amd/csrc/fy_rm2.hip
+++ b/filmyou-core_amd/csrc/fy_rm2.hip
@@ -263,17 +263,18 @@
     for (int64_t q = blockIdx.x * (int64_t)blockDim.x + threadIdx.x; q < nnz; q += (int64_t)gridDim.x * blockDim.x) out[q] = pair_rank[csc_pair[q]];
 }
 
-__device__ __forceinline__ void pack_csr_body(int32_t f0, int32_t f1, int32_t CH, const int32_t* __restrict__ csr_idx, const float* __restrict__ csr_r,
-                                              uint32_t* __restrict__ pk) {
+__device__ __forceinline__ void pack_csr_body(int32_t f0, int32_t f1, int32_t CH, int32_t planes, const int32_t* __restrict__ csr_idx,
+                                              const float* __restrict__ csr_r, uint32_t* __restrict__ pk) {
+    const int quarter = cooc_acc_quarter(planes != 0, CH);
     for (int64_t f = f0 + blockIdx.x * (int64_t)blockDim.x + threadIdx.x; f < f1; f += (int64_t)gridDim.x * blockDim.x)
-        pk[f] = (uint32_t)(csr_idx[f] % CH) | ((uint32_t)__half_as_ushort(__float2half(csr_r[f])) << 16);
-}
-__global__ void k_pack_csr(int32_t f0, int32_t f1, int32_t CH, const int32_t* __restrict__ csr_idx, const float* __restrict__ csr_r,
+        pk[f] = (uint32_t)cooc_acc_index(csr_idx[f] % CH, quarter) | ((uint32_t)__half_as_ushort(__float2half(csr_r[f])) << 16);
+}
+__global__ void k_pack_csr(int32_t f0, int32_t f1, int32_t CH, int32_t planes, const int32_t* __restrict__ csr_idx, const float* __restrict__ csr_r,
                            uint32_t* __restrict__ pk) {
-    pack_csr_body(f0, f1, CH, csr_idx, csr_r, pk);
-}
-
-__device__ __forceinline__ void tail_blocks_body(int32_t slot_base, int32_t n_slots, int32_t p_eff, const int32_t* __restrict__ rowptr,
+    pack_csr_body(f0, f1, CH, planes, csr_idx, csr_r, pk);
+}
+
+__device__ __forceinline__ void tail_blocks_body(int32_t slot_base, int32_t n_slots, int32_t p_eff, int32_t acc_quarter, const int32_t* __restrict__ rowptr,
                                                 const int32_t* __restrict__ csr_idx, const float* __restrict__ csr_r, uint32_t* __restrict__ y_pk,
                                                 int32_t* __restrict__ co2) {
     __shared__ int sh_count;
@@ -298,7 +299,7 @@
             if (start) {
                 float m = csr_r[f];
                 for (int32_t g = f + 1; g < end && ((csr_idx[g] - p_eff) >> 6) == blk; g++) m = fmaxf(m, csr_r[g]);
-                y_pk[base + at + __popcll(bal & ((1ull << lane) - 1ull))] = (uint32_t)blk | ((uint32_t)__half_as_ushort(__float2half(m)) << 16);
+                y_pk[base + at + __popcll(bal & ((1ull << lane) - 1ull))] = (uint32_t)cooc_acc_index(blk, acc_quarter) | ((uint32_t)__half_as_ushort(__float2half(m)) << 16);
             }
         }
         __syncthreads();
@@ -306,10 +307,10 @@
         __syncthreads();
     }
 }
-__global__ __launch_bounds__(256) void k_tail_blocks(int32_t slot_base, int32_t n_slots, int32_t p_eff, const int32_t* __restrict__ rowptr,
+__global__ __launch_bounds__(256) void k_tail_blocks(int32_t slot_base, int32_t n_slots, int32_t p_eff, int32_t acc_quarter, const int32_t* __restrict__ rowptr,
                                                      const int32_t* __restrict__ csr_idx, const float* __restrict__ csr_r, uint32_t* __restrict__ y_pk,
                                                      int32_t* __restrict__ co2) {
-    tail_blocks_body(slot_base, n_slots, p_eff, rowptr, csr_idx, csr_r, y_pk, co2);
+    tail_blocks_body(slot_base, n_slots, p_eff, acc_quarter, rowptr, csr_idx, csr_r, y_pk, co2);
 }
 
 __global__ void k_csr_values(int32_t nU, const int32_t* __restrict__ rowptr, const int32_t* __restrict__ csr_idx,
@@ -579,6 +580,7 @@
 struct CoDesc {
     int32_t slot_base, n_slots, CH, nch, f0, f1, p_eff, has_tail;
     int64_t co_off, co_tail_off;
+    int32_t planes, tail_width;
 };
 __global__ void k_chunk_offsets_multi(const CoDesc* __restrict__ D, const int32_t* __restrict__ rowptr, const int32_t* __restrict__ csr_idx,
                                       int32_t* __restrict__ co_all) {
@@ -587,13 +589,13 @@
 }
 __global__ void k_pack_csr_multi(const CoDesc* __restrict__ D, const int32_t* __restrict__ csr_idx, const float* __restrict__ csr_r, uint32_t* __restrict__ pk) {
     const CoDesc d = D[blockIdx.y];
-    pack_csr_body(d.f0, d.f1, d.CH, csr_idx, csr_r, pk);
+    pack_csr_body(d.f0, d.f1, d.CH, d.planes, csr_idx, csr_r, pk);
 }
 __global__ __launch_bounds__(256) void k_tail_blocks_multi(const CoDesc* __restrict__ D, const int32_t* __restrict__ rowptr, const int32_t* __restrict__ csr_idx,
                                                            const float* __restrict__ csr_r, uint32_t* __restrict__ y_pk, int32_t* __restrict__ co_tail_all) {
     const CoDesc d = D[blockIdx.y];
     if (!d.has_tail) return;
-    tail_blocks_body(d.slot_base, d.n_slots, d.p_eff, rowptr, csr_idx, csr_r, y_pk, co_tail_all + d.co_tail_off);
+    tail_blocks_body(d.slot_base, d.n_slots, d.p_eff, cooc_acc_quarter(d.planes != 0, d.tail_width), rowptr, csr_idx, csr_r, y_pk, co_tail_all + d.co_tail_off);
 }
 __global__ void k_csr_samples(int64_t n_samples, const int32_t* __restrict__ csr_idx, int32_t* __restrict__ samp) {
     for (int64_t k = blockIdx.x * (int64_t)blockDim.x + threadIdx.x; k < n_samples; k += (int64_t)gridDim.x * blockDim.x) samp[k] = csr_idx[k << FY_SAMPLE_SHIFT];
@@ -802,8 +804,10 @@
         const int c0 = (id & 255) * A.CH;
         const int row_of_item = A.row0 + (id >> 8) * (A.row_stride ? A.row_stride : 1);
         const int rmask = (cooc_row_is_cut(A, row_of_item) && row_of_item >= c0 && row_of_item < c0 + A.CH) ? row_of_item - c0 : -1;
-        if constexpr (PK) cooc_accumulate_pk<ACC>(A, acc, s0, s1, batch, rmask);
-        else cooc_accumulate_segments<false, ACC>(A, acc, s0, s1, c0, batch, rmask);
+        if constexpr (PK) {
+            if (__builtin_amdgcn_readfirstlane(rmask) >= 0) cooc_accumulate_pk<ACC, true>(A, acc, s0, s1, batch, cooc_acc_index(rmask, A.acc_quarter));
+            else cooc_accumulate_pk<ACC, false>(A, acc, s0, s1, batch);
+        } else cooc_accumulate_segments<false, ACC>(A, acc, s0, s1, c0, batch, rmask);
         if (threadIdx.x == 0) { sh_item = next; sh_s0 = se_next.x; sh_s1 = se_next.y; sh_id = id_next; }
         __syncthreads();
         const int nitem = sh_item;
@@ -1152,6 +1156,7 @@
     bool have_x = false;
     DevBuf<float> csc_x, csc_x_over_s;
     DevBuf<uint32_t> csr_pk, y_pk;
+    int32_t pk_planes = 0;
     DevBuf<int32_t> csc_rank, samples;
     std::vector<SegTable> segs, segs_tail;
     DevBuf<int32_t> g_co, g_co_tail, g_cnt, g_ptr, g_start;
@@ -1239,7 +1244,9 @@
                             int32_t* counter, hipStream_t st) {
     if (n_items <= 0) return;
     CoocArgs CA = CA_;
-    CA.acc_quarter = tune.cooc_planes ? cooc_lds_columns(CA.CH) / 4 : 0;
+    CA.acc_quarter = cooc_acc_quarter(tune.cooc_planes, CA.CH);
+    if (use_pk && CA.pk_layout != (tune.cooc_planes ? 2 : 1))
+        FY_FAIL(FY_ERR_STATE, "internal: the packed CSR holds layout %d, the row kernel's launch wants %d", CA.pk_layout, tune.cooc_planes ? 2 : 1);
     const bool acc32 = CA.acc32 && use_pk && CA.fx_scale > 0.0 && !tune.cooc_f32;
     const size_t lds = (size_t)cooc_lds_columns(CA.CH) * ((tune.cooc_f32 || acc32) ? 4 : 8);
     const int by_lds = (int)std::max<size_t>(1, (160 * 1024 - 512) / (lds + 64));
@@ -1281,7 +1288,7 @@
     EventTimer t_tab(ctx), t_walk(ctx);
     const size_t s0 = t_tab.begin();
     DevBuf<uint32_t> csr_pk(ctx, (size_t)P.nnz);
-    k_pack_csr<<<grid_for(P.nnz), 256, 0, st>>>(0, (int32_t)P.nnz, CH, P.csr_idx.get(), P.csr_r.get(), csr_pk.get());
+    k_pack_csr<<<grid_for(P.nnz), 256, 0, st>>>(0, (int32_t)P.nnz, CH, tune.cooc_planes ? 1 : 0, P.csr_idx.get(), P.csr_r.get(), csr_pk.get());
     FY_KERNEL_CHECK();
     DevBuf<int32_t> co(ctx, (size_t)P.nU * (nch + 1)), csc_rank(ctx, (size_t)P.nnz);
     build_chunk_offsets(ctx, P.rowptr.get(), P.csr_idx.get(), 0, P.nU, CH, nch, co.get(), st);
@@ -1294,6 +1301,7 @@
     CoocArgs CA{P.rank_pair.get(), P.pair_start.get(), segs.ptr.get(), segs.seg.get(), segs.w.get(), P.csr_idx.get(), nullptr, 0, 0, Ic, CH, nch,
                 0, Ic, 0, (int32_t)P.nnz, nullptr, 0, csr_pk.get(), nullptr, (uint32_t)std::min<int64_t>((int64_t)P.nnz * 4, 0xFFFFFFFFll)};
     CA.half = 1;
+    CA.pk_layout = tune.cooc_planes ? 2 : 1;
     CA.fx_scale = std::ldexp(1.0, fxk);
     CA.acc32 = acc32 ? 1 : 0;
     const int n_items = (int)cooc_item_count(Ic, CH, nch, true);
@@ -1329,7 +1337,9 @@
             FY_FAIL(FY_ERR_STATE, "internal: launch %zu of %zu of a batched row kernel has a null operand (item_seg %p item_id %p M %p seg %p ptr %p Bmax64 %p)", k, L.size(),
                     (const void*)L[k].A.item_seg, (const void*)L[k].A.item_id, (const void*)L[k].E.M, (const void*)L[k].A.seg, (const void*)L[k].A.seg_ptr, (const void*)L[k].E.Bmax64);
     for (auto& x : L) {
-        x.A.acc_quarter = tune.cooc_planes ? cooc_lds_columns(x.A.CH) / 4 : 0;
+        x.A.acc_quarter = cooc_acc_quarter(tune.cooc_planes, x.A.CH);
+        if (x.A.pk_layout != (tune.cooc_planes ? 2 : 1))
+            FY_FAIL(FY_ERR_STATE, "internal: the packed CSR holds layout %d, the batched row kernel's launch wants %d", x.A.pk_layout, tune.cooc_planes ? 2 : 1);
         max_chp = std::max(max_chp, cooc_lds_columns(x.A.CH));
         max_items = std::max(max_items, x.n_items);
         max_list = std::max(max_list, x.A.nrows * x.A.nch);
@@ -1414,7 +1424,8 @@
     for (size_t pi = 0; pi < np; pi++) {
         const Plan& p = plans[pi];
         const bool tail = p.p_eff < p.Ic;
-        hco[pi] = CoDesc{p.sbase, p.Uc, p.CH, p.nch, csr_range[2 * pi], csr_range[2 * pi + 1], p.p_eff, tail ? 1 : 0, co_total, co_tail_total};
+        hco[pi] = CoDesc{p.sbase, p.Uc, p.CH, p.nch, csr_range[2 * pi], csr_range[2 * pi + 1], p.p_eff, tail ? 1 : 0, co_total, co_tail_total,
+                         tc.pk_planes, p.tail_width};
         SegDesc m{p.sbase, p.q0, p.nq, p.nch, p.CH, (p.half || p.psym) ? 1 : 0, 0, p.nch + 1, co_total, cnt_total, 0, p.psym ? p.p_eff : 0,
                   p.psym ? 0 : p.p_eff, (p.panel && p.tail_chunks > 0 && p.p_eff < p.Ic) ? p.tail_chunks : 0};
         main_of[pi] = (int64_t)hsd.size();
@@ -2102,6 +2113,7 @@
         }
         std::vector<int32_t> sig;
         sig.push_back(use_pk ? 1 : 0);
+        sig.push_back(tune.cooc_planes ? 1 : 0);
         sig.push_back(plans.size() > 1 && !any_coop ? 1 : 0);
         for (auto& p : plans) {
             const int32_t v[8] = {p.c, p.CH, p.nch, p.half ? 1 : 0, p.panel ? 1 : 0, p.p_eff, p.tail_chunks, (p.coop ? 1 : 0) | (p.flat ? 2 : 0) | (p.psym ? 4 : 0)};
@@ -2117,6 +2129,7 @@
             segs.resize(plans.size());
             segs_tail.resize(plans.size());
             csr_pk.alloc(ctx, use_pk ? (size_t)P.nnz : 1);
+            tc.pk_planes = tune.cooc_planes ? 1 : 0;
             y_pk.alloc(ctx, any_tail ? (size_t)P.nnz : 1);
             csc_rank.alloc(ctx, any_half ? (size_t)P.nnz : 1);
             if (any_half) {
@@ -2140,7 +2153,7 @@
             const Plan& p = plans[pi];
             const int32_t f0 = csr_range[2 * pi], f1 = csr_range[2 * pi + 1];
             if (use_pk && f1 > f0) {
-                k_pack_csr<<<grid_for(f1 - f0), 256, 0, ts>>>(f0, f1, p.CH, P.csr_idx.get(), P.csr_r.get(), csr_pk.get());
+                k_pack_csr<<<grid_for(f1 - f0), 256, 0, ts>>>(f0, f1, p.CH, tc.pk_planes, P.csr_idx.get(), P.csr_r.get(), csr_pk.get());
                 FY_KERNEL_CHECK();
             }
             if (p.coop) return;
@@ -2150,7 +2163,8 @@
             build_segments(ctx, P.csc_slot.get(), use_pk ? csc_x_over_s.get() : csc_x.get(), co, p.sbase, p.q0, p.nq, p.nch, segs[pi], ts,
                            p.half ? csc_rank.get() : nullptr, P.csr_idx.get(), p.CH, nullptr, 0, seg_bound, p.half ? tc.samples.get() : nullptr);
             if (p.p_eff < p.Ic) {
-                k_tail_blocks<<<std::min<int>(p.Uc, ctx->num_cus * 16), 256, 0, ts>>>(p.sbase, p.Uc, p.p_eff, P.rowptr.get(), P.csr_idx.get(), P.csr_r.get(),
+                k_tail_blocks<<<std::min<int>(p.Uc, ctx->num_cus * 16), 256, 0, ts>>>(p.sbase, p.Uc, p.p_eff, cooc_acc_quarter(tc.pk_planes != 0, p.tail_width),
+                                                                          P.rowptr.get(), P.csr_idx.get(), P.csr_r.get(),
                                                                           y_pk.get(), co);
                 FY_KERNEL_CHECK();
                 build_segments(ctx, P.csc_slot.get(), csc_x_over_s.get(), co, p.sbase, p.q0, p.nq, 1, segs_tail[pi], ts, nullptr, nullptr, 0,
@@ -2210,6 +2224,7 @@
                                 csr_x.get(), p.pbase, p.sbase, p.Ic, p.CH, p.nch, 0, p.Ic, p.q0, p.nq, nullptr, 0, csr_pk.get(), nullptr,
                                 (uint32_t)std::min<int64_t>((int64_t)P.nnz * 4, 0xFFFFFFFFll)};
                     const int fxk = fx_exponent(&J->fx_bounds[3 * (size_t)c]);
+                    CA.pk_layout = tc.pk_planes + 1;
                     CA.fx_scale = std::ldexp(1.0, fxk);
                     const double w2s = (1.0 - lambda) * (1.0 - lambda) * (double)h_gscale[(size_t)c];
                     MEpilogue ME{Mc, p.ldm, (float)w2s, std::ldexp(w2s, -fxk), p.pack24 ? 1 : 0, nullptr, p.ldb, 0, 0, nullptr, p.ldb64, nullptr};
@@ -2395,7 +2410,7 @@
             const bool pack24 = p.pack24;
             if (p.coop) {
                 CoopShared X{J, R.get(), &tune, b_rank32.get(), a_rank.get(), use_pk ? csc_x_over_s.get() : csc_x.get(), csr_x.get(), csr_e.get(), csr_q.get(),
-                             use_pk ? csr_pk.get() : nullptr,
+                             use_pk ? csr_pk.get() : nullptr, tc.pk_planes + 1,
                              n_out.get(), out_off.get(), pvpi.get(), lo, &t_cooc, &t_score, &t_topn, prune_counters.get(),
                              &prune_blocks_total, &prune_seed_terms_cols, &coop_survived, &coop_pair_contribs, d_cshift.get(), h_gscale[(size_t)c]};
                 score_cluster_coop(X, p, ls);
@@ -2411,6 +2426,7 @@
                         csr_x.get(), pbase, sbase, Ic, CH, nch, 0, Ic, p.q0, p.nq, nullptr, 0, use_pk ? csr_pk.get() : nullptr, nullptr,
                         (uint32_t)std::min<int64_t>((int64_t)P.nnz * 4, 0xFFFFFFFFll)};
             const int fxk = (use_pk && tune.cooc_fx && !J->fx_bounds.empty()) ? fx_exponent(&J->fx_bounds[3 * (size_t)c]) : -1;
+            CA.pk_layout = tc.pk_planes + 1;
             CA.fx_scale = fxk >= 0 ? std::ldexp(1.0, fxk) : 0.0;
             const double w2s = (1.0 - lambda) * (1.0 - lambda) * (double)h_gscale[(size_t)c];
             MEpilogue ME{L.M.get(), ldm, (float)w2s, fxk >= 0 ? std::ldexp(w2s, -fxk) : 0.0,
@@ -2449,6 +2465,7 @@
                 CoocArgs CB{P.rank_pair.get(), P.pair_start.get(), segs_tail[pi].ptr_(), segs_tail[pi].seg_(), segs_tail[pi].w_(), P.csr_idx.get(),
                             csr_x.get(), pbase, sbase, Ic, p.tail_width, 1, p.p_eff, Ic - p.p_eff, p.q0, p.nq, nullptr, 0, y_pk.get(), nullptr, CA.pk_bytes};
                 CB.fx_scale = CA.fx_scale;
+                CB.pk_layout = tc.pk_planes + 1;
                 MEpilogue MB{reinterpret_cast<float*>(reinterpret_cast<char*>(PP.Bmax64) + (size_t)(p.p_eff / 64) * 3), p.tail_width, ME.w2, ME.fx_inv, 1,
                              nullptr, 0, 0, 0, nullptr, 0, nullptr, p.ldb64, 1};
                 int2* const tseg = batched ? plane[pi].item_seg_t.get() : L.item_seg.get();
diff --git a/filmyou-core_amd/csrc/fy_rm2_coop.hpp b/filmyou-core_amd/csrc/fy_rm2_coop.hpp
--- a/filmyou-core_amd/csrc/fy_rm2_coop.hpp
+++ b/filmyou-core_amd/csrc/fy_rm2_coop.hpp
@@ -7,6 +7,7 @@
     const float *b_rank;
     const float *a_rank, *csc_x, *csr_x, *csr_e, *csr_q;
     const uint32_t* csr_pk;
+    int32_t pk_layout;
     const int32_t *n_out, *out_off;
     const double* pvpi;
     int32_t lo;
@@ -116,6 +117,7 @@
                         X.csr_x, pbase, sbase, Ic, CH, nch, r0, nrows, 0, (int32_t)my_ratings, local_start.get(), W, X.csr_pk, nullptr,
                         (uint32_t)std::min<int64_t>((int64_t)P.nnz * 4, 0xFFFFFFFFll)};
             const int fxk = (X.csr_pk && tune.cooc_fx && !J->fx_bounds.empty()) ? fx_exponent(&J->fx_bounds[3 * (size_t)p.c]) : -1;
+            CA.pk_layout = X.pk_layout;
             CA.fx_scale = fxk >= 0 ? std::ldexp(1.0, fxk) : 0.0;
             const double w2s = (1.0 - lambda) * (1.0 - lambda) * (double)X.gscale;
             MEpilogue ME{const_cast<float*>(Mshift), ldm, (float)w2s, fxk >= 0 ? std::ldexp(w2s, -fxk) : 0.0,
```

After: 403.4 million, median of 6. About the same (+0.1%).
